# lelecaruso/NavierStokes_Project_NM4PDE

Hardware: AMD Instinct MI355X
Metric: time-steps/sec (assemble_time_step + solve_time_step), 3D flow past a cylinder, P2/P1, Yosida, per-rank ILU(0) (higher is better)
Workload: dtype f64

## Files before the change

include/nsx_host.h:

```cpp
#ifndef NSX_HOST_H
#define NSX_HOST_H

#include <stdint.h>

#ifdef __cplusplus
extern "C" {
#endif

typedef struct nsxh_mesh nsxh_mesh;
typedef struct nsxh_dofs nsxh_dofs;
typedef struct nsxh_tables nsxh_tables;


nsxh_mesh *nsxh_mesh_cylinder(int dim, int m, int nr, int nxu, int nxd, int nyb, int nyt, int nz,
                              double grade_x, double grade_r);
nsxh_mesh *nsxh_mesh_cylinder_level(int dim, int level);
nsxh_mesh *nsxh_mesh_cube(int n);
nsxh_mesh *nsxh_mesh_box(int dim, int nx, int ny, int nz, const double *lo, const double *hi);
nsxh_mesh *nsxh_mesh_read_msh(const char *path);
void nsxh_mesh_free(nsxh_mesh *);

int nsxh_mesh_dim(const nsxh_mesh *);
int nsxh_mesh_n_vertices(const nsxh_mesh *);
int nsxh_mesh_n_cells(const nsxh_mesh *);
// ... 2 lines not shown
const int32_t *nsxh_mesh_cells(const nsxh_mesh *);
const int32_t *nsxh_mesh_bfaces(const nsxh_mesh *);
const int32_t *nsxh_mesh_bface_ids(const nsxh_mesh *);
const int32_t *nsxh_mesh_bface_cells(const nsxh_mesh *);
const int32_t *nsxh_mesh_subdomain(const nsxh_mesh *);

int nsxh_mesh_partition(nsxh_mesh *, int n_parts, int n_sub);
int nsxh_mesh_partition_owned(nsxh_mesh *, int n_parts, int n_sub);


nsxh_dofs *nsxh_distribute_dofs(const nsxh_mesh *);
enum { NSXH_ORDER_FIRST_TOUCH = 0, NSXH_ORDER_COLOUR = 1, NSXH_ORDER_COLOUR_ALL = 2 };
nsxh_dofs *nsxh_distribute_dofs_ordered(const nsxh_mesh *, int ordering);
int nsxh_n_colours(const nsxh_dofs *);
int nsxh_n_colours_p(const nsxh_dofs *);
void nsxh_dofs_free(nsxh_dofs *);

int nsxh_dofs_per_cell(const nsxh_dofs *);
int nsxh_n_nodes_p2(const nsxh_dofs *);
int nsxh_n_nodes_p1(const nsxh_dofs *);
int nsxh_n_u(const nsxh_dofs *);
int nsxh_n_p(const nsxh_dofs *);
const int32_t *nsxh_cell_dofs(const nsxh_dofs *);
const double *nsxh_cell_coords(const nsxh_dofs *);
const double *nsxh_support_points(const nsxh_dofs *);
const int32_t *nsxh_node_owner(const nsxh_dofs *);
const int32_t *nsxh_pnode_owner(const nsxh_dofs *);
const int32_t *nsxh_owned_u_ptr(const nsxh_dofs *);
const int32_t *nsxh_owned_p_ptr(const nsxh_dofs *);
int nsxh_n_subdomains(const nsxh_dofs *);

int nsxh_boundary_dofs(nsxh_dofs *, int boundary_id, const int32_t **dofs);

int nsxh_reference_sparsity(nsxh_dofs *, int block, const int32_t **rowptr, const int32_t **colind);

typedef struct nsxh_rank_view nsxh_rank_view;
nsxh_rank_view *nsxh_rank_view_create(const nsxh_dofs *, int rank, int world);
void nsxh_rank_view_free(nsxh_rank_view *);
int nsxh_rank_view_n_cells(const nsxh_rank_view *);
int nsxh_rank_view_n_cells_layer1(const nsxh_rank_view *);
const int32_t *nsxh_rank_view_cell_ids(const nsxh_rank_view *);
const int32_t *nsxh_rank_view_cell_dofs(const nsxh_rank_view *);
const double *nsxh_rank_view_cell_coords(const nsxh_rank_view *);
const int32_t *nsxh_rank_view_gpu_u_ptr(const nsxh_rank_view *);
const int32_t *nsxh_rank_view_gpu_p_ptr(const nsxh_rank_view *);
int nsxh_rank_view_n_virtual_ranks(const nsxh_rank_view *);
const int32_t *nsxh_rank_view_rank_u_ptr(const nsxh_rank_view *);
const int32_t *nsxh_rank_view_rank_p_ptr(const nsxh_rank_view *);
int nsxh_rank_view_n_neighbors(const nsxh_rank_view *);
const int32_t *nsxh_rank_view_neighbors(const nsxh_rank_view *);
const int32_t *nsxh_rank_view_send_u_ptr(const nsxh_rank_view *);
const int32_t *nsxh_rank_view_send_u_nodes(const nsxh_rank_view *);
const int32_t *nsxh_rank_view_send_p_ptr(const nsxh_rank_view *);
const int32_t *nsxh_rank_view_send_p_nodes(const nsxh_rank_view *);


nsxh_tables *nsxh_tables_create(int dim, int rule, int order);
void nsxh_tables_free(nsxh_tables *);
int nsxh_tables_n_q(const nsxh_tables *);
int nsxh_tables_n_p2(const nsxh_tables *);
int nsxh_tables_n_p1(const nsxh_tables *);
const double *nsxh_tables_points(const nsxh_tables *);
const double *nsxh_tables_weights(const nsxh_tables *);
const double *nsxh_tables_N2(const nsxh_tables *);
const double *nsxh_tables_dN2(const nsxh_tables *);
const double *nsxh_tables_N1(const nsxh_tables *);
const double *nsxh_tables_dN1(const nsxh_tables *);
int nsxh_tables_n_qf(const nsxh_tables *);


int nsxh_write_vtu(const nsxh_dofs *, const double *solution, const char *directory, const char *basename, unsigned counter);

int nsxh_pressure_difference(const nsxh_dofs *, const double *solution, const double *point_a, const double *point_b, double *diff);


int nsxh_ilu_stream_stats(int n_rows, const int32_t *rowptr, const int32_t *colind, int n_blocks, const int32_t *block_ptr,
                          int blocks_per_wave, int ncomp, int gap, int entries_per_tick, int64_t out[6]);
int nsxh_ilu_stream_apply(int n_rows, const int32_t *rowptr, const int32_t *colind, int n_blocks, const int32_t *block_ptr,
                          int blocks_per_wave, int ncomp, int gap, int entries_per_tick, const double *lu, const double *b, double *x);

int nsxh_ilu_stream_apply_f32(int n_rows, const int32_t *rowptr, const int32_t *colind, int n_blocks, const int32_t *block_ptr,
                              int blocks_per_wave, int ncomp, int gap, int entries_per_tick, const double *lu, const double *b, double *x);

int nsxh_internal_layout(int dim, int n_cells, int dofs_per_cell, const int32_t *cell_dofs, const double *cell_coords, int n_u, int n_p,
                         int n_in_ranks, const int32_t *in_u_ptr, const int32_t *in_p_ptr, int n_virtual, int order, int schur_max_rows,
                         int32_t *node_perm, int32_t *pnode_perm, int32_t *n_ranks, int32_t *u_ptr, int32_t *p_ptr, int32_t *n_schur,
                         int32_t *schur_ptr, int32_t *colours);

#ifdef __cplusplus
}
#endif
#endif
```

navierstokes_project_nm4pde_amd/csrc/nsx_blas.hip:

```cpp
#include "nsx_grid.hpp"
#include "nsx_ilu_lanes.hpp"

namespace nsx {

constexpr int RED_BLOCKS = 512;
constexpr int RED_STRIDE = 1024;

struct SRef {
  double c;
  int num, den;
  int num_nb, den_nb;
};

__device__ __forceinline__ double wave_sum_all(double v) {
#pragma unroll
  for (int o = 32; o > 0; o >>= 1) v += __shfl_xor(v, o, 64);
  return v;
}

__device__ __forceinline__ double slot_value(const double *__restrict__ scal, const double *__restrict__ partial, int slot, int nb,
                                             double *sh) {
  if (nb == 0) return scal[slot];
  if (threadIdx.x < 64) {
    const double *p = partial + (size_t)slot * RED_STRIDE;
// ... 315 lines not shown
  const unsigned long long seq = ++h->pub_seq;
  unsigned long long *flag_dev = (unsigned long long *)(h->pub_dev + N_SLOTS);
  hipLaunchKernelGGL(k_publish, dim3(count), dim3(256), 0, h->stream, slot0, count, args, h->red_partial.p, h->scal.p, h->pub_dev, flag_dev, seq,
                     h->pub_counter.p);
  return seq;
}
void collect_published(nsx_handle *h, unsigned long long seq, int slot0, int count, double *out) {
  wait_published(h, seq);
  for (int i = 0; i < count; ++i) out[i] = h->pub_host[slot0 + i];
}
void read_scalars(nsx_handle *h, int slot0, int count, double *out) { collect_published(h, publish_scalars(h, slot0, count), slot0, count, out); }
void write_scalar(nsx_handle *h, int slot, double v) {
  HIP_CHECK(hipStreamSynchronize(h->stream));
  h->scal_host[slot] = v;
  h->slot_nb[slot] = 0;
  HIP_CHECK(hipMemcpyAsync(h->scal.p + slot, h->scal_host + slot, sizeof(double), hipMemcpyHostToDevice, h->stream));
  HIP_CHECK(hipStreamSynchronize(h->stream));
}

int cg_dirty_words(nsx_handle *h);

}

extern "C" int nsx_persistent_state(nsx_handle *h, int state[4]) {
  if (!h || !state) return NSX_ERR_ARG;
  try {
    HIP_CHECK(hipSetDevice(h->prm.device));
    state[0] = h->mgs.box.p != nullptr && !h->mgs.disabled && h->mgs.max_wg > 0;
    state[1] = h->cg_box.p != nullptr && !h->cg_disabled && h->cg_max_wg > 0;
    state[2] = h->n_persistent_fallbacks;
    state[3] = nsx::mgs_dirty_words(h) + nsx::cg_dirty_words(h);
  } catch (const nsx::Error &e) {
    h->err = e.msg;
    return e.code;
  }
  return NSX_OK;
}

extern "C" int nsx_path_info(nsx_handle *h, int info[32]) {
  if (!h || !info) return NSX_ERR_ARG;
  for (int k = 0; k < 32; ++k) info[k] = 0;
  if (!h->have_mesh) return NSX_OK;
  try {
    HIP_CHECK(hipSetDevice(h->prm.device));
    const nsx::SpmvBlocked &b = h->blkA;
    info[0] = nsx::blocked_usable(h) ? 1 : 0;
    info[1] = b.n_chunks;
    info[2] = b.n_chunks_if;
    info[3] = h->mgs.last_e;
    info[4] = h->mgs.last_nwg;
    info[5] = h->mgs.last_dist;
    info[6] = h->mgs.max_e_seen;
    info[7] = h->cu_reserved;
    info[8] = h->cg_last_path;
    info[9] = h->schedS.n_blocks;
    info[10] = (int)h->haloU.nbr.size();
    info[11] = h->haloU.nbr.empty() ? 0 : h->haloU.send_ptr[h->haloU.nbr.size()];
    info[12] = h->N2_loc - h->N2;
    info[13] = h->schedS.dense ? 1 : 0;
    info[14] = h->mgs.disabled ? 1 : 0;
    info[15] = h->n_persistent_fallbacks;
    if (!h->mgs.disabled) {
      nsx::mgs_setup(h);
      const int es[3] = {8, 10, 12};
      auto fit = [&](int n, const int *caps, int n_inst) {
        const nsx::MgsPick p = nsx::mgs_pick(n, caps, n_inst, es);
        return p.fits() ? p.e : 0;
      };
      info[16] = fit(h->n_u, h->mgs.max_wg_dist, 1);
      info[17] = fit(h->n_u, h->mgs.dist_cap_reserved, 3);
      info[18] = fit(h->n_u + h->n_p, h->mgs.max_wg_dist, 1);
      info[19] = fit(h->n_u + h->n_p, h->mgs.dist_cap_reserved, 3);
      info[21] = fit(h->n_u, h->mgs.max_wg_e, 3);
    }
    info[20] = nsx::cdiv(std::max(1, h->schedS.n_blocks), 1024);
    info[22] = h->N2;
    info[23] = h->NP;
    info[24] = h->mgs.last_fused;
    info[25] = h->mgs.fused_launches;
    info[26] = h->inner_F_fp32_used;
    info[27] = h->ilu_F_fp32_used;
    info[28] = h->cg_last_rpg;
    info[29] = h->cg_last_lres;
  } catch (const nsx::Error &e) {
    h->err = e.msg;
    return e.code;
  }
  return NSX_OK;
}
```

navierstokes_project_nm4pde_amd/csrc/nsx_internal.hpp:

```cpp
#pragma once
#include <hip/hip_runtime.h>

#include <cstdint>
#include <cstdio>
#include <cstring>
#include <map>
#include <string>
#include <functional>
#include <vector>

#include "../../include/nsx.h"
#include "../host/graph.hpp"

#ifndef NSX_NT
#define NSX_NT 1
#endif
template <int BIT, class T>
__device__ __forceinline__ T ld_stream(const T *p) {
  if constexpr ((NSX_NT & BIT) != 0) return __builtin_nontemporal_load(p);
  else return *p;
}

namespace nsx {

// ... 157 lines not shown
  int max_wg_e[3] = {0, 0, 0};
  int max_wg_dist[3] = {0, 0, 0};
  int dist_cap_reserved[3] = {0, 0, 0};
  int links = 0;
  bool disabled = false;
  double guard_override = -1.0;
  DevBuf<double> ls_partial, ls_vals, ls_gram;
  int ls_mode = -1;
  DevBuf<double> ext_vals;
  DevBuf<unsigned long long> ext_words;
  unsigned int ext_expected = 0;
  int ext_parity = 0;
  bool redo_ahead = false;
  int dist_state = -1;
  std::map<int, int> dist_fit;
  bool leave_req = false;
  int local_timeouts = 0;
  int ilu_cap[3] = {-1, -1, -1}, ilu_cap_rows = -1;
  int last_e = 0, last_nwg = 0, last_dist = 0, max_e_seen = 0;
  int last_fused = 0, fused_launches = 0;
};

struct Comm;

enum { N_SLOTS = 128 };

}

struct nsx_handle {
  nsx_params prm{};
  std::string err;
  hipStream_t stream = nullptr;
  int dim = 0, n_q = 0, np2 = 0, np1 = 0, dpc = 0;
  int n_cells = 0, N2 = 0, NP = 0, n_u = 0, n_p = 0;
  int N2_loc = 0, NP_loc = 0;
  int n_cells1 = 0;
  int g_u = 0, g_p = 0, off_p = 0, len_blk = 0, len_u = 0, len_p = 0;
  bool dist = false;
  int rank = 0, world = 1, goff_u = 0, goff_p = 0, n_u_glob = 0, n_p_glob = 0;
  std::vector<int32_t> ghost_u, ghost_p;
  nsx::HaloPlan haloU, haloP;
  nsx::RowSplit splitA, splitVel, splitB, splitG, splitS;
  hipStream_t comm_stream = nullptr;
  hipEvent_t ev_ready = nullptr;
  bool have_tables = false, have_mesh = false, assembled = false, prec_ready = false;
  std::vector<double> N2_h, dN2_h, N1_h, w_h;
  nsx::DevBuf<double> tab_N2, tab_dN2, tab_N1, tab_w, tab_N2T, tab_dN2T;
  nsx::DevBuf<int32_t> cell_n2, cell_n1;
  nsx::DevBuf<double> geo;
  std::vector<int32_t> cell_n2_h, cell_n1_h;
  std::vector<int32_t> cell_n2_in, cell_n1_in;
  std::vector<double> cell_coords_in;
  std::vector<int32_t> in_rank_u_h, in_rank_p_h, in_sblk_h;
  int layout_req_ranks = 0, layout_req_order = 0, layout_req_schur = 0;
  bool layout_on = false;
  int layout_colours = 0, layout_colours_p = 0;
  std::vector<int32_t> perm2_h, perm1_h, iperm2_h, iperm1_h;
  nsx::DevBuf<int32_t> perm2_d, perm1_d;
  nsx::DevBuf<double> io_stage;
  nsx::Csr caller_graph[2];
  std::vector<int32_t> caller_pos[2];
  nsx::DevCsr gA, gG, gB, gS, gPM;
  nsx::SpmvBlocked blkA;
  nsx::DevBuf<double> vS0, vMass, vStiff, vConv, vF, vG, vB, vPM, vSchur, luF, luS;
  int inner_precision = NSX_INNER_FP64;
  nsx::DevBuf<float> vF32;
  int inner_F_fp32_used = 0, ilu_F_fp32_used = 0;
  nsx::DevBuf<int32_t> bt_of_g;
  nsx::GatherMap gmA, gmG, gmB, gmPM;
  nsx::DevBuf<double> cellbuf;
  nsx::DevBuf<double> sol, sol_owned, prev_sol, rhs;
  std::vector<int32_t> rank_u_h, rank_p_h, sblk_h;
  nsx::DevBuf<int32_t> rank_u;
  nsx::IluSchedule schedF, schedS;
  nsx::DevBuf<double> dbar;
  nsx::DevBuf<int32_t> bc_dofs;
  nsx::DevBuf<double> bc_vals;
  nsx::DevBuf<double> dirmask;
  std::vector<int32_t> bc_cache;
  nsx::DevBuf<double> diag_D, diag_D_inv, neg_diag_D_inv, lump_M, schur_w;
  nsx::DevBuf<double> schur_w_prev;
  bool schur_valid = false, schur_pending = false;
  int schur_type = -1;
  std::vector<nsx::DevBuf<double> *> pool;
  nsx::DevBuf<double> red_partial;
  nsx::DevBuf<double> scal;
  int slot_nb[nsx::N_SLOTS] = {0};
  double *scal_host = nullptr;
  double *pub_host = nullptr, *pub_dev = nullptr;
  unsigned long long pub_seq = 0;
  nsx::DevBuf<unsigned int> pub_counter;
  nsx::MgsState mgs;
  bool sched_dirty = true;
  int gx_drop_wg = -1;
  int n_persistent_fallbacks = 0;
  int gmres_depth = 0;
  bool cu_reserve_failed = false;
  int cgd_agreed = -1;
  nsx::DevBuf<double> ext_self;
  hipStream_t stream_plain = nullptr;
  std::vector<hipStream_t> retired_streams;
  int cu_reserved = 0;
  int comm_probe_local = -1;
  long long n_allreduce = 0, n_halo = 0;
  int self_p2p = 0;
  int n_ext_collectives = 0;
  nsx::DevBuf<unsigned long long> cg_box;
  nsx::CgPlan cgplan;
  nsx::DevBuf<double> cg_vec;
  int cg_parity = 0, cg_max_wg = 0, cg_max_wg_res[2] = {0, 0};
  int cg_max_wg_lres[2] = {0, 0};
  bool cg_resident = false;
  bool cg_lds_resident = false;
  bool cg_variant_said = false;
  bool cg_disabled = false;
  nsx::DevBuf<double> cgd_raw;
  int cg_last_path = 0;
  int cg_last_rpg = 0, cg_last_lres = 0;
  nsx::DevBuf<double> cgd_vec, cgd_parts;
  int ff_n = 0, ff_nq = 0;
  nsx::DevBuf<int32_t> ff_cells, ff_lf;
  nsx::DevBuf<double> ff_N2, ff_dN2, ff_N1, ff_w, ff_out;
  nsx::DevBuf<uint8_t> diag_counted;
  int diag_n_counted = 0;
  nsx::DevBuf<double> diag_planes;
  nsx::DevBuf<double> diag_fold;
  nsx::DevBuf<double> diag_max;
  bool diag_valid = false;
  bool prof_on = false;
  std::map<std::string, nsx::ProfEntry> prof;
  std::vector<std::string> prof_names;
  nsx::Comm *comm = nullptr;
  bool defer_red = false;
  std::vector<int> pending_red;
};

namespace nsx {

struct LaunchScope {
  nsx_handle *h;
  ProfEntry *e = nullptr;
  hipEvent_t a = nullptr, b = nullptr;
  LaunchScope(nsx_handle *h_, const char *name, double bytes) : h(h_) {
    if (!h->prof_on) return;
    e = &h->prof[name];
    e->bytes += bytes;
    (void)hipEventCreate(&a);
    (void)hipEventCreate(&b);
    (void)hipEventRecord(a, h->stream);
  }
  ~LaunchScope() {
    if (!e) return;
    (void)hipEventRecord(b, h->stream);
    e->launches++;
    e->pending.emplace_back(a, b);
  }
};

inline int cdiv(int64_t a, int64_t b) { return (int)((a + b - 1) / b); }

void setup_ilu_schedule(nsx_handle *h, const Csr &g, const std::vector<int32_t> &block_ptr, IluSchedule &s, int blocks_per_wave, bool allow_dense = false,
                        int ncomp = 1);
void build_schur_graph(nsx_handle *h);
void vec_from_caller(nsx_handle *h, double *dev, const double *host, bool with_ghosts);
void vec_to_caller(nsx_handle *h, const double *dev, double *host);
void part_from_caller(nsx_handle *h, int which, double *dev, const double *host);
void part_to_caller(nsx_handle *h, int which, const double *dev, double *host);
void pressure_from_caller(nsx_handle *h, double *dev, const double *host);
void pressure_to_caller(nsx_handle *h, const double *dev, double *host);
inline int32_t node_to_internal(const nsx_handle *h, int32_t local_node) { return h->layout_on ? h->perm2_h[local_node] : local_node; }
inline int32_t pnode_to_internal(const nsx_handle *h, int32_t local_node) { return h->layout_on ? h->perm1_h[local_node] : local_node; }
void ensure_schedules(nsx_handle *h);

void run_assemble(nsx_handle *h, bool first, int flags);
void run_dirichlet(nsx_handle *h, int n, const int32_t *dofs, const double *vals);

void diag_mesh_setup(nsx_handle *h);

bool blocked_usable(const nsx_handle *h);
void spmv_F(nsx_handle *h, const double *vals, const double *x, double *y, const float *vals32 = nullptr, const double *rb = nullptr);
void spmv_F_inner(nsx_handle *h, const double *x, double *y);
void spmv_F_inner_resid(nsx_handle *h, const double *x, const double *b, double *y);
void convert_F_f32(nsx_handle *h);
void spmv_saddle(nsx_handle *h, const double *x, double *y);
void spmv_G(nsx_handle *h, const double *xp, double *yu, bool accumulate);
void spmv_B(nsx_handle *h, const double *xu, double *yp, const double *r = nullptr, int sub = 0);
void spmv_S(nsx_handle *h, const double *x, double *y);
void schur_numeric(nsx_handle *h, const double *w);
void ilu_factor(nsx_handle *h, const DevCsr &g, IluSchedule &s, const double *vals, double *lu, const char *name, bool f32 = false);
void ilu_check(nsx_handle *h);
bool ilu_solve(nsx_handle *h, const DevCsr &g, const IluSchedule &s, const double *lu, const double *b, double *x, int ncomp,
               const char *name, int dot_slot = -1, bool f32 = false, int *used_f32 = nullptr);
void extract_diag(nsx_handle *h, const DevCsr &g, const double *vals, double *d);
void abs_rowsum(nsx_handle *h, const DevCsr &g, const double *vals, double *d);

struct Span {
  int n, split, gap;
  Span(int n_) : n(n_), split(n_), gap(0) {}
  Span(int n_, int split_, int gap_) : n(n_), split(split_), gap(gap_) {}
};
inline Span blk_span(const nsx_handle *h) { return Span(h->n_u + h->n_p, h->n_u, h->g_u); }

template <int CTRL>
__device__ __forceinline__ double dpp_f64(double v) {
  int lo = __double2loint(v), hi = __double2hiint(v);
  lo = __builtin_amdgcn_update_dpp(0, lo, CTRL, 0xf, 0xf, true);
  hi = __builtin_amdgcn_update_dpp(0, hi, CTRL, 0xf, 0xf, true);
  return __hiloint2double(hi, lo);
}
template <int CTRL, int ROW_MASK>
__device__ __forceinline__ double dpp_f64_rows(double v) {
  int lo = __double2loint(v), hi = __double2hiint(v);
  lo = __builtin_amdgcn_update_dpp(0, lo, CTRL, ROW_MASK, 0xf, false);
  hi = __builtin_amdgcn_update_dpp(0, hi, CTRL, ROW_MASK, 0xf, false);
  return __hiloint2double(hi, lo);
}

void v_copy(nsx_handle *h, int n, double *d, const double *s);
void v_zero(nsx_handle *h, int n, double *d);
void v_add(nsx_handle *h, Span n, double *d, double a, const double *v);
void v_add_dev(nsx_handle *h, Span n, double *d, double a, int slot, const double *v);
void v_sadd(nsx_handle *h, Span n, double *d, double s, double a, const double *v);
void v_scale(nsx_handle *h, Span n, double *d, double a);
void v_scale_dev_inv(nsx_handle *h, Span n, double *d, int slot);
void v_scale_vec(nsx_handle *h, int n, double *d, const double *f);
void v_dot(nsx_handle *h, Span n, const double *a, const double *b, int slot);
void v_add_and_dot(nsx_handle *h, Span n, double *d, double a, int aslot, const double *v, const double *w, int slot);
bool v_mgs(nsx_handle *h, Span n, double *w, int dim, double *const *vs, int slot0, bool normalize, double *out,
           const std::function<void()> *after_launch = nullptr, bool consider = false, double *gram = nullptr, const double *ilu_rhs = nullptr);
void v_axpy_multi(nsx_handle *h, Span n, double *x, int k, double *const *vs, const double *coef_host);
void v_axpy_multi_into(nsx_handle *h, Span n, double *x, const double *x0, const double *y, int k, double *const *vs, const double *coef_host);
void finalize_slots(nsx_handle *h, int slot0, int count);
double *red_out(nsx_handle *h, int slot, int nb);
void after_reduction(nsx_handle *h, int slot, int nb);
int red_blocks(nsx_handle *h, int n);
__device__ __forceinline__ double block_sum_256(double v, double *sh) {
#pragma unroll
  for (int o = 32; o > 0; o >>= 1) v += __shfl_down(v, o, 64);
  const int w = threadIdx.x >> 6, l = threadIdx.x & 63;
  if (l == 0) sh[w] = v;
  __syncthreads();
  double t = 0.0;
  if (threadIdx.x == 0) {
    for (int k = 0; k < (int)(blockDim.x >> 6); ++k) t += sh[k];
  }
  return t;
}
void defer_reductions(nsx_handle *h, bool on);
double read_scalar(nsx_handle *h, int slot);
void read_scalars(nsx_handle *h, int slot0, int count, double *out);
unsigned long long publish_scalars(nsx_handle *h, int slot0, int count);
void collect_published(nsx_handle *h, unsigned long long seq, int slot0, int count, double *out);
void wait_published(nsx_handle *h, unsigned long long seq);
void mgs_setup(nsx_handle *h);
int mgs_dirty_words(nsx_handle *h);
struct MgsPick {
  int e = 0, nwg = 1, per_thread = 1 << 30;
  bool fits() const { return e != 0 && per_thread <= e; }
};
MgsPick mgs_pick(int n, const int *caps, int n_inst, const int *es);
void build_cg_plan(nsx_handle *h);
void cg_pack_values(nsx_handle *h);
bool cg_schur_persistent(nsx_handle *h, double *x, const double *b, double rtol, int maxiter, int *steps, double *last, int *status);
bool cg_schur_fused(nsx_handle *h, double *x, const double *b, double rtol, int maxiter, int *steps, double *last, int *status);
void write_scalar(nsx_handle *h, int slot, double v);

void prec_initialize(nsx_handle *h, int type);
void prec_confirm(nsx_handle *h);
void prec_vmult(nsx_handle *h, int type, double inner_rtol, int inner_maxiter, double *dst, const double *src,
                nsx_solve_stats *st, bool fused);
void solve_time_step(nsx_handle *h, int type, double tol, double inner_rtol, int maxiter, int inner_maxiter,
                     nsx_solve_stats *st);

void comm_allreduce_scalars(nsx_handle *h, int slot0, int count);
void comm_allreduce_partials(nsx_handle *h, double *partials, int count);
bool comm_agree_all(nsx_handle *h, bool mine);
// ... 17 lines not shown
```

navierstokes_project_nm4pde_amd/csrc/nsx_setup.hip:

```cpp
#include <algorithm>
#include <cmath>
#include <numeric>

#include "nsx_internal.hpp"
#include "../host/ilu_stream.hpp"
#include "../host/layout.hpp"

using namespace nsx;

static thread_local std::string g_create_error;

namespace nsx {

static void upload_csr(nsx_handle *h, DevCsr &d, bool square) {
  d.rowptr.upload(d.host.rowptr, h->stream);
  d.colind.upload(d.host.colind, h->stream);
  if (square) {
    std::vector<int32_t> diag(d.host.n_rows);
    for (int32_t i = 0; i < d.host.n_rows; ++i) {
      diag[i] = find_in_row(d.host, i, i);
      if (diag[i] < 0) NSX_THROW(NSX_ERR_ARG, "square graph has no diagonal entry in row %d", i);
    }
    d.diag.upload(diag, h->stream);
  }
}

static void build_gather(nsx_handle *h, const Csr &g, int n_cells, int per_r, const int32_t *cell_r, int per_c,
                         const int32_t *cell_c, int plane_stride, bool plane_rc_swapped, GatherMap &gm) {
  const int64_t nnz = g.nnz();
  std::vector<int32_t> ptr(nnz + 1, 0);
  std::vector<int32_t> epos((size_t)n_cells * per_r * per_c);
  for (int c = 0; c < n_cells; ++c)
    for (int a = 0; a < per_r; ++a)
      for (int b = 0; b < per_c; ++b) {
        const int32_t row = cell_r[(size_t)c * per_r + a];
        if (row >= g.n_rows) {
          epos[((size_t)c * per_r + a) * per_c + b] = -1;
          continue;
        }
        const int32_t e = find_in_row(g, row, cell_c[(size_t)c * per_c + b]);
        if (e < 0) NSX_THROW(NSX_ERR_ARG, "internal: cell pair not in graph");
        epos[((size_t)c * per_r + a) * per_c + b] = e;
        ptr[e + 1]++;
      }
  for (int64_t e = 0; e < nnz; ++e) ptr[e + 1] += ptr[e];
  std::vector<int32_t> src(ptr[nnz]);
  std::vector<int32_t> fill(ptr.begin(), ptr.end() - 1);
  for (int c = 0; c < n_cells; ++c)
    for (int a = 0; a < per_r; ++a)
      for (int b = 0; b < per_c; ++b) {
        const int32_t e = epos[((size_t)c * per_r + a) * per_c + b];
        if (e < 0) continue;
        const int64_t plane = plane_rc_swapped ? ((int64_t)b * per_r + a) : ((int64_t)a * per_c + b);
        const int64_t off = plane * plane_stride * n_cells + c;
        if (off > INT32_MAX) NSX_THROW(NSX_ERR_UNSUPPORTED, "mesh too large for int32 gather offsets");
        src[fill[e]++] = (int32_t)off;
      }
  gm.n_out = nnz;
  gm.n_src = (int64_t)src.size();
  gm.ptr.upload(ptr, h->stream);
  gm.src.upload(src, h->stream);
}

void setup_ilu_schedule(nsx_handle *h, const Csr &g, const std::vector<int32_t> &bptr, IluSchedule &s, int blocks_per_wave, bool allow_dense, int ncomp) {
  const int nb = (int)bptr.size() - 1;
  s.n_blocks = nb;
  s.block_ptr_h = bptr;
  s.max_rows = 0;
  std::vector<int32_t> lev(g.n_rows, 0);
  std::vector<int32_t> f_ptr{0}, f_rows, b_ptr{0}, b_rows, off_f(nb + 1, 0), off_b(nb + 1, 0);
  f_rows.reserve(g.n_rows);
  b_rows.reserve(g.n_rows);
  s.max_levels = 0;
  std::vector<std::vector<int32_t>> buckets;
  for (int b = 0; b < nb; ++b) {
    const int r0 = bptr[b], r1 = bptr[b + 1];
    s.max_rows = std::max(s.max_rows, r1 - r0);
    for (int pass = 0; pass < 2; ++pass) {
      int nl = 0;
      if (pass == 0) {
        for (int i = r0; i < r1; ++i) {
          int l = 0;
          for (int k = g.rowptr[i]; k < g.rowptr[i + 1]; ++k) {
            const int j = g.colind[k];
            if (j >= i) break;
            if (j >= r0) l = std::max(l, lev[j] + 1);
          }
          lev[i] = l;
          nl = std::max(nl, l + 1);
// ... 214 lines not shown
    b.grid_if = 0;
    b.frac_if = g.nnz() ? (double)nnz_second / (double)g.nnz() : 0.0;
    if (!second.empty()) make_desc(second, b.desc_if, b.grid_if, nullptr);
  }
  b.crow.upload(bounds, h->stream);
  b.cptr.upload(cptr, h->stream);
  b.ucols.upload(ucols, h->stream);
  b.lidx.upload(lidx, h->stream);
  if (getenv("NSX_DEBUG"))
    fprintf(stderr, "[nsx] blocked spmv: rows %d chunks %d (max %d rows; %d of them stage a ghost column: %.1f %% of the non-zeros) unique cols/chunk avg %.0f max %d (nnz/unique %.1f)\n",
            g.n_rows, b.n_chunks, b.max_rows, b.n_chunks_if, 100.0 * b.frac_if, b.ucols_total / std::max(1, b.n_chunks), b.max_ucols, (double)g.nnz() / b.ucols_total);
}

static std::vector<int32_t> spmv_chunks(nsx_handle *h) {
  const int n = h->gA.host.n_rows;
  const int target = getenv("NSX_SPMV_R") ? std::max(16, std::min(448, atoi(getenv("NSX_SPMV_R")))) : 130;
  std::vector<int32_t> bounds{0};
  const std::vector<int32_t> &rk = h->rank_u_h;
  const bool by_rank = !(getenv("NSX_SPMV_BY_RANK") && atoi(getenv("NSX_SPMV_BY_RANK")) == 0) && rk.size() > 2 &&
                       (double)n / (double)(rk.size() - 1) <= target;
  const bool split_ranks = !by_rank && !(getenv("NSX_SPMV_BY_RANK") && atoi(getenv("NSX_SPMV_BY_RANK")) == 0) && rk.size() > 2 &&
                           (double)n / (double)(rk.size() - 1) <= 4.0 * target;
  if (by_rank) {
    int start = 0;
    for (size_t r = 1; r < rk.size(); ++r) {
      if (rk[r] - start > target && rk[r - 1] > start) {
        bounds.push_back(rk[r - 1]);
        start = rk[r - 1];
      }
    }
    bounds.push_back(n);
  } else if (split_ranks) {
    for (size_t r = 0; r + 1 < rk.size(); ++r) {
      const int rows = rk[r + 1] - rk[r];
      if (rows <= 0) continue;
      const int parts = (rows + target - 1) / target;
      for (int q = 1; q <= parts; ++q) bounds.push_back(rk[r] + (int)((int64_t)rows * q / parts));
    }
    if (bounds.back() != n) bounds.push_back(n);
  } else {
    for (int r = 128; r < n; r += 128) bounds.push_back(r);
    bounds.push_back(n);
  }
  std::vector<int32_t> out{0};
  for (size_t c = 1; c < bounds.size(); ++c) {
    while (bounds[c] - out.back() > 448) out.push_back(out.back() + 224);
    if (bounds[c] > out.back()) out.push_back(bounds[c]);
  }
  return out;
}

void build_schur_graph(nsx_handle *h) {
  const Csr &B = h->gB.host;
  std::vector<int32_t> tp((size_t)h->N2_loc + 1, 0), tr(B.nnz());
  for (int64_t k = 0; k < B.nnz(); ++k) tp[B.colind[k] + 1]++;
  for (int i = 0; i < h->N2_loc; ++i) tp[i + 1] += tp[i];
  {
    std::vector<int32_t> fill(tp.begin(), tp.end() - 1);
    for (int j = 0; j < B.n_rows; ++j)
      for (int k = B.rowptr[j]; k < B.rowptr[j + 1]; ++k) tr[fill[B.colind[k]]++] = j;
  }
  Csr S;
  S.n_rows = h->NP;
  S.n_cols = h->NP_loc;
  S.rowptr.assign((size_t)h->NP + 1, 0);
  std::vector<int32_t> mark(h->NP_loc, -1), cols;
  for (int i = 0; i < h->NP; ++i) {
    cols.clear();
    for (int kb = B.rowptr[i]; kb < B.rowptr[i + 1]; ++kb) {
      const int k = B.colind[kb];
      for (int q = tp[k]; q < tp[k + 1]; ++q) {
        const int j = tr[q];
        if (mark[j] != i) {
          mark[j] = i;
          cols.push_back(j);
        }
      }
    }
    std::sort(cols.begin(), cols.end());
    S.colind.insert(S.colind.end(), cols.begin(), cols.end());
    S.rowptr[i + 1] = (int32_t)S.colind.size();
  }
  h->gS.host = std::move(S);
  upload_csr(h, h->gS, true);
  h->vSchur.alloc(h->gS.nnz());
  h->luS.alloc(h->gS.nnz());
}

static void default_ranks(nsx_handle *h) {
  h->in_rank_u_h = {0, h->N2};
  h->in_rank_p_h = {0, h->NP};
  h->in_sblk_h.clear();
}

static void refresh_rank_products(nsx_handle *h) {
  h->rank_u.upload(h->rank_u_h, h->stream);
  h->dbar.alloc(h->rank_u_h.size() - 1);
  h->sched_dirty = true;
  h->prec_ready = false;
  h->schur_valid = false;
  h->mgs.dist_fit.clear();
}

void ensure_schedules(nsx_handle *h) {
  if (!h->sched_dirty) return;
  build_blocked(h, h->gA.host, spmv_chunks(h), h->blkA, h->N2);
  auto blocks_per_wave = [](int n_rows, size_t n_blocks) { return std::max(1, std::min(64, (int)(680.0 * (double)n_blocks / std::max(1, n_rows) + 0.5))); };
  const std::vector<int32_t> &sb = h->sblk_h.empty() ? h->rank_p_h : h->sblk_h;
  const int bpwF = getenv("NSX_BPW_F") ? atoi(getenv("NSX_BPW_F")) : blocks_per_wave(h->N2, h->rank_u_h.size() - 1);
  const int bpwS = getenv("NSX_BPW_S") ? atoi(getenv("NSX_BPW_S")) : blocks_per_wave(h->NP, sb.size() - 1);
  setup_ilu_schedule(h, h->gA.host, h->rank_u_h, h->schedF, bpwF, false, h->dim);
  const bool denseS = !(getenv("NSX_DENSE_S") && atoi(getenv("NSX_DENSE_S")) == 0);
  setup_ilu_schedule(h, h->gS.host, sb, h->schedS, bpwS, denseS, 1);
  build_cg_plan(h);
  h->cgd_agreed = -1;
  h->sched_dirty = false;
}


__global__ void k_perm_vec(int n, int ncomp, const int32_t *__restrict__ perm, double *caller, double *internal, int to_internal) {
  const int i = blockIdx.x * blockDim.x + threadIdx.x;
  if (i >= n) return;
  const int node = i / ncomp, c = i - node * ncomp;
  const int64_t j = (int64_t)perm[node] * ncomp + c;
  if (to_internal) internal[j] = caller[i];
  else caller[i] = internal[j];
}

static void perm_launch(nsx_handle *h, int which, double *caller_dev, double *internal_dev, bool to_internal) {
  const int ncomp = which == 0 ? h->dim : 1, n = which == 0 ? h->n_u : h->n_p;
  if (n) hipLaunchKernelGGL(k_perm_vec, dim3(cdiv(n, 256)), dim3(256), 0, h->stream, n, ncomp, (which == 0 ? h->perm2_d : h->perm1_d).p, caller_dev, internal_dev, to_internal ? 1 : 0);
}

void part_from_caller(nsx_handle *h, int which, double *dev, const double *host) {
  const int n = which == 0 ? h->n_u : h->n_p;
  if (!h->layout_on) {
    HIP_CHECK(hipMemcpyAsync(dev, host, (size_t)n * sizeof(double), hipMemcpyHostToDevice, h->stream));
  } else {
    h->io_stage.alloc((size_t)h->n_u + h->n_p);
    HIP_CHECK(hipMemcpyAsync(h->io_stage.p, host, (size_t)n * sizeof(double), hipMemcpyHostToDevice, h->stream));
    perm_launch(h, which, h->io_stage.p, dev, true);
  }
  HIP_CHECK(hipStreamSynchronize(h->stream));
}

void part_to_caller(nsx_handle *h, int which, const double *dev, double *host) {
  const int n = which == 0 ? h->n_u : h->n_p;
  if (!h->layout_on) {
    HIP_CHECK(hipMemcpyAsync(host, dev, (size_t)n * sizeof(double), hipMemcpyDeviceToHost, h->stream));
  } else {
    h->io_stage.alloc((size_t)h->n_u + h->n_p);
    perm_launch(h, which, h->io_stage.p, const_cast<double *>(dev), false);
    HIP_CHECK(hipMemcpyAsync(host, h->io_stage.p, (size_t)n * sizeof(double), hipMemcpyDeviceToHost, h->stream));
  }
  HIP_CHECK(hipStreamSynchronize(h->stream));
}

void pressure_from_caller(nsx_handle *h, double *dev, const double *host) {
  if (!h->dist) return part_from_caller(h, 1, dev, host);
  std::vector<double> loc(h->len_p, 0.0);
  for (int i = 0; i < h->NP; ++i) loc[pnode_to_internal(h, i)] = host[(size_t)h->goff_p + i];
  HIP_CHECK(hipMemcpyAsync(dev, loc.data(), loc.size() * sizeof(double), hipMemcpyHostToDevice, h->stream));
  HIP_CHECK(hipStreamSynchronize(h->stream));
}
void pressure_to_caller(nsx_handle *h, const double *dev, double *host) {
  if (!h->dist) return part_to_caller(h, 1, dev, host);
  std::vector<double> loc(h->n_p);
  HIP_CHECK(hipMemcpyAsync(loc.data(), dev, loc.size() * sizeof(double), hipMemcpyDeviceToHost, h->stream));
  HIP_CHECK(hipStreamSynchronize(h->stream));
  for (int i = 0; i < h->NP; ++i) host[(size_t)h->goff_p + i] = loc[pnode_to_internal(h, i)];
}

void vec_from_caller(nsx_handle *h, double *dev, const double *host, bool with_ghosts) {
  const int dim = h->dim;
  if (!h->dist) {
    if (!h->layout_on) {
      HIP_CHECK(hipMemcpyAsync(dev, host, ((size_t)h->n_u + h->n_p) * sizeof(double), hipMemcpyHostToDevice, h->stream));
    } else {
      h->io_stage.alloc((size_t)h->n_u + h->n_p);
      HIP_CHECK(hipMemcpyAsync(h->io_stage.p, host, ((size_t)h->n_u + h->n_p) * sizeof(double), hipMemcpyHostToDevice, h->stream));
      perm_launch(h, 0, h->io_stage.p, dev, true);
      perm_launch(h, 1, h->io_stage.p + h->n_u, dev + h->off_p, true);
    }
    HIP_CHECK(hipStreamSynchronize(h->stream));
    return;
  }
  std::vector<double> loc(h->len_blk, 0.0);
  for (int i = 0; i < h->N2; ++i)
    for (int c = 0; c < dim; ++c) loc[(size_t)dim * node_to_internal(h, i) + c] = host[(size_t)dim * (h->goff_u + i) + c];
  for (int i = 0; i < h->NP; ++i) loc[h->off_p + pnode_to_internal(h, i)] = host[(size_t)h->n_u_glob + h->goff_p + i];
  if (with_ghosts) {
    for (size_t g = 0; g < h->ghost_u.size(); ++g)
      for (int c = 0; c < dim; ++c) loc[h->n_u + g * dim + c] = host[(size_t)dim * h->ghost_u[g] + c];
    for (size_t g = 0; g < h->ghost_p.size(); ++g) loc[h->off_p + h->n_p + g] = host[(size_t)h->n_u_glob + h->ghost_p[g]];
  }
  HIP_CHECK(hipMemcpyAsync(dev, loc.data(), loc.size() * sizeof(double), hipMemcpyHostToDevice, h->stream));
  HIP_CHECK(hipStreamSynchronize(h->stream));
// ... 773 lines not shown
```

navierstokes_project_nm4pde_amd/csrc/nsx_solve.hip:

```cpp
#include <chrono>
#include <cmath>
#include <functional>
#include <memory>

#include "nsx_internal.hpp"

namespace nsx {

void cg_update(nsx_handle *h, int n, double *x, const double *d, double *g, const double *hv, int gh_slot, int dh_slot, int res_slot);
void cg_direction(nsx_handle *h, int n, double *d, const double *hv, int num_slot, int den_slot);
void v_reciprocal(nsx_handle *h, int n, double *d, const double *s, double num);

struct Tmp {
  nsx_handle *h;
  DevBuf<double> *b;
  Tmp(nsx_handle *h_, size_t n) : h(h_), b(nullptr) {
    for (size_t i = 0; i < h->pool.size(); ++i)
      if (h->pool[i]->n >= n) {
        b = h->pool[i];
        h->pool.erase(h->pool.begin() + i);
        break;
      }
    if (!b) {
      b = new DevBuf<double>();
// ... 221 lines not shown
}

using OpDot = std::function<bool(double *dst, const double *src, int slot)>;
static SolveResult cg(nsx_handle *h, const Op &A, double *x, const double *b, const Op &P, Span n, int len, double tol, int maxiter,
                      const OpDot *Pdot = nullptr) {
  auto apply_P_dot = [&](double *dst, const double *src, int slot) {
    if (Pdot && (*Pdot)(dst, src, slot)) return;
    if (!Pdot) P(dst, src);
    v_dot(h, n, src, dst, slot);
  };
  SolveResult res{1, 0, 0.0};
  Tmp g(h, len), d(h, len), hv(h, len);
  int it = 0;
  A(g.p(), x);
  v_add(h, n, g.p(), -1., b);
  v_dot(h, n, g.p(), g.p(), S_RES);
  double r = std::sqrt(read_scalar(h, S_RES));
  res.last = r;
  int conv = sc_check(0, r, tol, maxiter);
  if (conv == 0) {
    int gh = S_GH, gh_new = S_GH2;
    apply_P_dot(hv.p(), g.p(), gh);
    v_copy(h, n.n, d.p(), hv.p());
    v_scale(h, n, d.p(), -1.);
    while (conv == 0) {
      it++;
      A(hv.p(), d.p());
      v_dot(h, n, d.p(), hv.p(), S_DH);
      const bool batch = h->comm != nullptr;
      DeferScope defer(h, batch);
      cg_update(h, n.n, x, d.p(), g.p(), hv.p(), gh, S_DH, S_RES);
      unsigned long long seq = 0;
      if (!batch) seq = publish_scalars(h, S_RES, 1);
      apply_P_dot(hv.p(), g.p(), gh_new);
      if (batch) {
        defer.release();
        seq = publish_scalars(h, S_RES, 1);
      }
      double res2;
      collect_published(h, seq, S_RES, 1, &res2);
      r = std::sqrt(std::fabs(res2));
      res.last = r;
      conv = sc_check(it, r, tol, maxiter);
      if (conv != 0) break;
      cg_direction(h, n.n, d.p(), hv.p(), gh_new, gh);
      std::swap(gh, gh_new);
    }
  }
  res.status = conv == 1 ? 0 : 1;
  res.steps = it;
  return res;
}

static double norm2(nsx_handle *h, Span n, const double *v) {
  v_dot(h, n, v, v, S_T);
  return std::sqrt(read_scalar(h, S_T));
}

static Op schur_product(nsx_handle *h) {
  return [h](double *d, const double *s) { spmv_S(h, s, d); };
}
static Op schur_ilu(nsx_handle *h) {
  return [h](double *d, const double *s) { ilu_solve(h, h->gS, h->schedS, h->luS.p, s, d, 1, "ilu_solve_S"); };
}

static SolveResult schur_cg(nsx_handle *h, double rtol, int maxit, double *x, const double *b) {
  int steps = 0, status = 0;
  double last = 0.0;
  h->cg_last_rpg = h->cg_last_lres = 0;
  if (cg_schur_persistent(h, x, b, rtol, maxit, &steps, &last, &status)) return SolveResult{status, steps, last};
  if (cg_schur_fused(h, x, b, rtol, maxit, &steps, &last, &status)) return SolveResult{status, steps, last};
  h->cg_last_path = 1;
  const Op Sm = schur_product(h), PS = schur_ilu(h);
  OpDot PSdot = [h](double *d, const double *s, int slot) { return ilu_solve(h, h->gS, h->schedS, h->luS.p, s, d, 1, "ilu_solve_S", slot); };
  return cg(h, Sm, x, b, PS, h->n_p, h->len_p, rtol * norm2(h, h->n_p, b), maxit, &PSdot);
}

__global__ void k_same_and_keep(int n, const double *__restrict__ w, double *__restrict__ prev, int *changed) {
  const int i = blockIdx.x * blockDim.x + threadIdx.x;
  if (i >= n) return;
  const unsigned long long a = (unsigned long long)__double_as_longlong(w[i]), b = (unsigned long long)__double_as_longlong(prev[i]);
  if (a != b) {
    prev[i] = w[i];
    __hip_atomic_store(changed, 1, __ATOMIC_RELAXED, __HIP_MEMORY_SCOPE_SYSTEM);
  }
}
static bool schur_inputs_unchanged(nsx_handle *h, int type) {
  const bool cache = !(getenv("NSX_SCHUR_CACHE") && atoi(getenv("NSX_SCHUR_CACHE")) == 0);
  const int n = h->len_u;
  volatile int *flag = (volatile int *)(h->pub_host + N_SLOTS + 4);
  const bool had = h->schur_valid && h->schur_type == type && (int)h->schur_w_prev.n == n;
  if (!had) {
    h->schur_w_prev.alloc(n);
    comm_halo_u(h, h->schur_w.p);
    v_copy(h, n, h->schur_w_prev.p, h->schur_w.p);
    return false;
  }
  comm_halo_u(h, h->schur_w.p);
  *flag = 0;
  hipLaunchKernelGGL(k_same_and_keep, dim3(cdiv(n, 256)), dim3(256), 0, h->stream, n, h->schur_w.p, h->schur_w_prev.p, (int *)(h->pub_dev + N_SLOTS + 4));
  HIP_CHECK(hipStreamSynchronize(h->stream));
  return cache && !h->comm && *flag == 0;
}

void prec_initialize(nsx_handle *h, int type) {
  ensure_schedules(h);
  if (!h->assembled) NSX_THROW(NSX_ERR_ARG, "assemble before initialising a preconditioner");
  HIP_CHECK(hipSetDevice(h->prm.device));
  const int n_u = h->n_u;
  const double *V = nullptr;
  if (type == NSX_PREC_YOSIDA) {
    extract_diag(h, h->gA, h->vMass.p, h->diag_D.p);
  } else if (type == NSX_PREC_SIMPLE || type == NSX_PREC_ASIMPLE || type == NSX_PREC_AYOSIDA) {
    extract_diag(h, h->gA, h->vF.p, h->diag_D.p);
  } else {
    NSX_THROW(NSX_ERR_ARG, "Invalid preconditioner type");
  }
  v_reciprocal(h, n_u, h->diag_D_inv.p, h->diag_D.p, 1.0);
  v_reciprocal(h, n_u, h->neg_diag_D_inv.p, h->diag_D.p, -1.0);
  V = h->neg_diag_D_inv.p;
  if (type == NSX_PREC_AYOSIDA) {
    abs_rowsum(h, h->gA, h->vMass.p, h->lump_M.p);
    v_reciprocal(h, n_u, h->lump_M.p, h->lump_M.p, -1.0);
    V = h->lump_M.p;
  }
  v_copy(h, n_u, h->schur_w.p, V);
  v_scale_vec(h, n_u, h->schur_w.p, h->dirmask.p);
  v_scale(h, n_u, h->schur_w.p, -1.0);
  const bool f32 = h->inner_precision == NSX_INNER_FP32;
  if (f32) convert_F_f32(h);
  ilu_factor(h, h->gA, h->schedF, h->vF.p, h->luF.p, "ilu_factor_F", f32);
  if (!schur_inputs_unchanged(h, type)) {
    h->schur_valid = false;
    h->schur_pending = true;
    schur_numeric(h, h->schur_w.p);
    cg_pack_values(h);
    ilu_factor(h, h->gS, h->schedS, h->vSchur.p, h->luS.p, "ilu_factor_S");
    h->schur_type = type;
  }
  h->prec_ready = true;
}

void prec_confirm(nsx_handle *h) {
  try {
    ilu_check(h);
  } catch (...) {
    h->schur_valid = false;
    h->schur_pending = false;
    h->prec_ready = false;
    throw;
  }
  if (h->schur_pending) {
    h->schur_pending = false;
    h->schur_valid = true;
  }
}

static void count(nsx_solve_stats *st, bool F, const SolveResult &r) {
  if (!st) return;
  if (F) {
    st->inner_F_iterations += r.steps;
    st->n_F_solves++;
  } else {
    st->inner_S_iterations += r.steps;
    st->n_S_solves++;
  }
  if (r.status) st->status = 2;
}

static bool step_fused() { return !(getenv("NSX_STEP_FUSED") && atoi(getenv("NSX_STEP_FUSED")) == 0); }

void prec_vmult(nsx_handle *h, int type, double tol, int maxit, double *dst, const double *src, nsx_solve_stats *st, bool fused) {
  if (!h->prec_ready) NSX_THROW(NSX_ERR_ARG, "preconditioner not initialised");
  const int n_u = h->n_u, n_p = h->n_p, dim = h->dim, len_u = h->len_u, len_p = h->len_p;
  const double *src_u = src, *src_p = src + h->off_p;
  double *dst_u = dst, *dst_p = dst + h->off_p;
  Op Fm = [h](double *d, const double *s) { spmv_F_inner(h, s, d); };
  const bool f32 = h->inner_precision == NSX_INNER_FP32;
  const Op Sm = schur_product(h), PS = schur_ilu(h);
  Op PF = [h, dim, f32](double *d, const double *s) {
    int used = 0;
    ilu_solve(h, h->gA, h->schedF, h->luF.p, s, d, dim, "ilu_solve_F", -1, f32, &used);
    if (used) h->ilu_F_fp32_used = 1;
  };
  auto cg_S = [&](double *x, const double *b) { return schur_cg(h, tol, maxit, x, b); };
  const ResidOp Fr = [h](double *d, const double *x, const double *b) { spmv_F_inner_resid(h, x, b, d); };
  auto solve_F = [&](double *x, const double *b, bool x_is_zero, Seams *sm) {
    if (!sm) return count(st, true, gmres(h, Fm, x, b, PF, n_u, len_u, tol * norm2(h, n_u, b), maxit, false, x_is_zero, true, true));
    sm->rtol = tol;
    sm->A_resid = &Fr;
    v_dot(h, n_u, b, b, S_T);
    count(st, true, gmres(h, Fm, x, b, PF, n_u, len_u, 0.0, maxit, false, x_is_zero, true, true, sm));
  };
  auto solve_F_from_src = [&](double *x) {
    if (!fused) return solve_F(x, src_u, false, nullptr);
    Seams sm;
    sm.x0 = src_u;
    solve_F(x, src_u, false, &sm);
    if (!sm.x_written) v_copy(h, n_u, x, src_u);
  };
  auto B_and_sub = [&](const double *x, double *out, const double *r, int sign) {
    if (fused) return spmv_B(h, x, out, r, sign);
    spmv_B(h, x, out);
    if (sign > 0) v_add(h, n_p, out, -1.0, r);
    else v_sadd(h, n_p, out, -1.0, 1.0, r);
  };
  std::unique_ptr<Tmp> own_u, own_p;
  double *yu = dst_u, *yp = dst_p;
  if (!fused && (type == NSX_PREC_YOSIDA || type == NSX_PREC_SIMPLE)) {
    own_u = std::make_unique<Tmp>(h, len_u);
    own_p = std::make_unique<Tmp>(h, len_p);
    yu = own_u->p();
    yp = own_p->p();
  }
// ... 245 lines not shown
```

navierstokes_project_nm4pde_amd/csrc/nsx_sparse.hip:

```cpp
#include <atomic>

#include "nsx_internal.hpp"
#include "nsx_ilu_lanes.hpp"

namespace nsx {

template <int LW>
__device__ __forceinline__ double lane_group_sum(double v) {
  if (LW >= 2) v += dpp_f64<0xB1>(v);
  if (LW >= 4) v += dpp_f64<0x4E>(v);
  if (LW >= 8) v += dpp_f64<0x141>(v);
  if (LW >= 16) v += dpp_f64<0x140>(v);
  if (LW >= 32) v += __shfl_xor(v, 16, 64);
  if (LW >= 64) v += __shfl_xor(v, 32, 64);
  return v;
}

template <int W>
__device__ __forceinline__ double group_sum(double v) {
  return lane_group_sum<W>(v);
}

template <int DIM, int W, bool WITH_G, bool RESID>
__device__ __forceinline__ void spmv_vel_rows(int n_rows, const int32_t *__restrict__ rp, const int32_t *__restrict__ ci,
                                              const double *__restrict__ av, const double *__restrict__ x,
                                              const int32_t *__restrict__ grp, const int32_t *__restrict__ gci,
                                              const double *__restrict__ gv, const double *__restrict__ xp,
                                              double *__restrict__ y, const int32_t *__restrict__ rows, const double *__restrict__ b) {
  const int bid = (blockIdx.x & 7) * (gridDim.x >> 3) + (blockIdx.x >> 3);
  const int slot = (bid * 256 + threadIdx.x) / W, lane = threadIdx.x % W;
  if (slot >= n_rows) return;
  const int row = rows ? rows[slot] : slot;
  double acc[DIM];
#pragma unroll
  for (int c = 0; c < DIM; ++c) acc[c] = 0.0;
  const int e = rp[row + 1];
  for (int p = rp[row] + lane; p < e; p += W) {
    const double a = av[p];
    const double *xj = x + (size_t)ci[p] * DIM;
#pragma unroll
    for (int c = 0; c < DIM; ++c) acc[c] += a * xj[c];
  }
  if (WITH_G) {
    const int ge = grp[row + 1];
    for (int p = grp[row] + lane; p < ge; p += W) {
      const double xk = xp[gci[p]];
#pragma unroll
      for (int c = 0; c < DIM; ++c) acc[c] += gv[(size_t)p * DIM + c] * xk;
    }
  }
#pragma unroll
  for (int c = 0; c < DIM; ++c) acc[c] = group_sum<W>(acc[c]);
  if (lane == 0) {
#pragma unroll
    for (int c = 0; c < DIM; ++c) y[(size_t)row * DIM + c] = RESID ? b[(size_t)row * DIM + c] - acc[c] : acc[c];
  }
}
template <int DIM, int W, bool WITH_G>
__global__ __launch_bounds__(256) void k_spmv_vel(int n_rows, const int32_t *__restrict__ rp, const int32_t *__restrict__ ci,
                                                  const double *__restrict__ av, const double *__restrict__ x,
                                                  const int32_t *__restrict__ grp, const int32_t *__restrict__ gci,
                                                  const double *__restrict__ gv, const double *__restrict__ xp,
                                                  double *__restrict__ y, const int32_t *__restrict__ rows) {
  spmv_vel_rows<DIM, W, WITH_G, false>(n_rows, rp, ci, av, x, grp, gci, gv, xp, y, rows, nullptr);
}
template <int DIM, int W>
__global__ __launch_bounds__(256) void k_spmv_vel_resid(int n_rows, const int32_t *__restrict__ rp, const int32_t *__restrict__ ci,
                                                        const double *__restrict__ av, const double *__restrict__ x, double *__restrict__ y,
                                                        const int32_t *__restrict__ rows, const double *__restrict__ b) {
  spmv_vel_rows<DIM, W, false, true>(n_rows, rp, ci, av, x, nullptr, nullptr, nullptr, nullptr, y, rows, b);
}

template <int DIM, int W>
__global__ __launch_bounds__(256) void k_spmv_G(int n_rows, const int32_t *__restrict__ rp, const int32_t *__restrict__ ci,
                                                const double *__restrict__ gv, const double *__restrict__ xp,
                                                double *__restrict__ y, int accumulate, const int32_t *__restrict__ rows) {
  const int slot = (blockIdx.x * 256 + threadIdx.x) / W, lane = threadIdx.x % W;
  if (slot >= n_rows) return;
  const int row = rows ? rows[slot] : slot;
  double acc[DIM];
#pragma unroll
  for (int c = 0; c < DIM; ++c) acc[c] = 0.0;
  const int e = rp[row + 1];
  for (int p = rp[row] + lane; p < e; p += W) {
    const double xk = xp[ci[p]];
#pragma unroll
// ... 389 lines not shown

void spmv_saddle(nsx_handle *h, const double *x, double *y) {
  double *xx = const_cast<double *>(x);
  if (h->dist) {
    comm_halo_begin(h, h->haloU, xx, h->dim);
    comm_halo_begin(h, h->haloP, xx + h->off_p, 1);
  }
  const bool blk_dist = h->dist && blocked_usable(h);
  {
    LaunchScope ls(h, "spmv_saddle_u", bytes_vel(h, true));
    if (blk_dist) launch_blocked(h, h->vF.p, x, y, 0);
    else if (h->dist) launch_vel(h, true, h->vF.p, x, x + h->off_p, y, h->splitVel.interior.p, h->splitVel.n_interior);
    else if (launch_blocked(h, h->vF.p, x, y)) launch_G(h, x + h->off_p, y, true, nullptr, h->N2);
    else launch_vel(h, true, h->vF.p, x, x + h->off_p, y, nullptr, h->N2);
  }
  {
    LaunchScope ls(h, "spmv_B", bytes_B(h));
    if (h->dist) launch_B(h, x, y + h->off_p, h->splitB.interior.p, h->splitB.n_interior);
    else launch_B(h, x, y + h->off_p, nullptr, h->NP);
  }
  if (h->dist) {
    {
      LaunchScope ls(h, "halo_up_wait", bytes_halo(h->haloU, h->dim) + bytes_halo(h->haloP, 1));
      comm_halo_finish(h, h->haloU, xx, h->dim);
      comm_halo_finish(h, h->haloP, xx + h->off_p, 1);
    }
    LaunchScope ls(h, "spmv_saddle_if", 0);
    if (blk_dist) {
      launch_blocked(h, h->vF.p, x, y, 1);
      launch_G(h, x + h->off_p, y, true, nullptr, h->N2);
    } else {
      launch_vel(h, true, h->vF.p, x, x + h->off_p, y, h->splitVel.interface.p, h->splitVel.n_interface);
    }
    launch_B(h, x, y + h->off_p, h->splitB.interface.p, h->splitB.n_interface);
  }
}

void spmv_S(nsx_handle *h, const double *x, double *y) {
  LaunchScope ls(h, "spmv_S", 12.0 * h->gS.nnz() + 20.0 * h->NP);
  if (h->dist) {
    double *xx = const_cast<double *>(x);
    comm_halo_begin(h, h->haloP, xx, 1);
    launch_S(h, x, y, h->splitS.interior.p, h->splitS.n_interior);
    comm_halo_finish(h, h->haloP, xx, 1);
    launch_S(h, x, y, h->splitS.interface.p, h->splitS.n_interface);
    return;
  }
  launch_S(h, x, y, nullptr, h->NP);
}

static void split_rows(nsx_handle *h, RowSplit &sp, int n_rows, const Csr &a, int own_a, const Csr *b, int own_b) {
  std::vector<int32_t> in, out;
  for (int i = 0; i < n_rows; ++i) {
    bool ghost = false;
    for (int k = a.rowptr[i]; k < a.rowptr[i + 1] && !ghost; ++k) ghost = a.colind[k] >= own_a;
    if (b)
      for (int k = b->rowptr[i]; k < b->rowptr[i + 1] && !ghost; ++k) ghost = b->colind[k] >= own_b;
    (ghost ? out : in).push_back(i);
  }
  sp.n_interior = (int)in.size();
  sp.n_interface = (int)out.size();
  sp.interior.upload(in, h->stream);
  sp.interface.upload(out, h->stream);
}
void build_row_splits(nsx_handle *h) {
  if (!h->dist) return;
  split_rows(h, h->splitA, h->N2, h->gA.host, h->N2, nullptr, 0);
  split_rows(h, h->splitVel, h->N2, h->gA.host, h->N2, &h->gG.host, h->NP);
  split_rows(h, h->splitG, h->N2, h->gG.host, h->NP, nullptr, 0);
  split_rows(h, h->splitB, h->NP, h->gB.host, h->N2, nullptr, 0);
  split_rows(h, h->splitS, h->NP, h->gS.host, h->NP, nullptr, 0);
  if (getenv("NSX_DEBUG"))
    fprintf(stderr, "[nsx] rank %d: interface rows F %d / %d, block(1,0) %d / %d, S %d / %d\n", h->rank, h->splitA.n_interface, h->N2, h->splitB.n_interface,
            h->NP, h->splitS.n_interface, h->NP);
}

void convert_F_f32(nsx_handle *h) {
  const int64_t n = h->gA.nnz();
  h->vF32.alloc((size_t)n);
  LaunchScope ls(h, "F_to_f32", 12.0 * (double)n);
  if (n > 0) hipLaunchKernelGGL(k_to_f32, dim3(cdiv(n, 256)), dim3(256), 0, h->stream, n, h->vF.p, h->vF32.p, (int *)(h->pub_dev + N_SLOTS + 3));
}

__global__ void k_extract_diag(int n_nodes, int dim, const int32_t *__restrict__ diag, const double *__restrict__ v, double *__restrict__ d) {
  const int i = blockIdx.x * blockDim.x + threadIdx.x;
  if (i >= n_nodes * dim) return;
  d[i] = v[diag[i / dim]];
}
__global__ void k_abs_rowsum(int n_nodes, int dim, const int32_t *__restrict__ rp, const double *__restrict__ v, double *__restrict__ d) {
  const int i = blockIdx.x * blockDim.x + threadIdx.x;
  if (i >= n_nodes) return;
  double s = 0.0;
  for (int p = rp[i]; p < rp[i + 1]; ++p) s += fabs(v[p]);
  for (int c = 0; c < dim; ++c) d[(size_t)i * dim + c] = s;
}
void extract_diag(nsx_handle *h, const DevCsr &g, const double *vals, double *d) {
  LaunchScope ls(h, "extract_diag", 0);
  hipLaunchKernelGGL(k_extract_diag, dim3(cdiv(h->n_u, 256)), dim3(256), 0, h->stream, g.n_rows(), h->dim, g.diag.p, vals, d);
}
void abs_rowsum(nsx_handle *h, const DevCsr &g, const double *vals, double *d) {
  LaunchScope ls(h, "abs_rowsum", 0);
  hipLaunchKernelGGL(k_abs_rowsum, dim3(cdiv(g.n_rows(), 256)), dim3(256), 0, h->stream, g.n_rows(), h->dim, g.rowptr.p, vals, d);
}

template <int DIM>
__global__ __launch_bounds__(64) void k_schur(int n_rows, const int32_t *__restrict__ srp, const int32_t *__restrict__ sci,
                                              const int32_t *__restrict__ brp, const int32_t *__restrict__ bci,
                                              const double *__restrict__ bv, const double *__restrict__ w, int max_row,
                                              double *__restrict__ sv) {
  extern __shared__ double smem[];
  double *rv = smem;
  int32_t *rc = (int32_t *)(smem + (size_t)max_row * DIM);
  const int i = blockIdx.x;
  if (i >= n_rows) return;
  const int b0 = brp[i], nb = brp[i + 1] - b0;
  for (int t = threadIdx.x; t < nb; t += 64) {
    const int k = bci[b0 + t];
    rc[t] = k;
#pragma unroll
    for (int c = 0; c < DIM; ++c) rv[t * DIM + c] = bv[(size_t)(b0 + t) * DIM + c] * w[(size_t)k * DIM + c];
  }
  __syncthreads();
  for (int e = srp[i] + threadIdx.x; e < srp[i + 1]; e += 64) {
    const int j = sci[e];
    double acc = 0.0;
    int q = 0;
    for (int p = brp[j]; p < brp[j + 1]; ++p) {
      const int k = bci[p];
      while (q < nb && rc[q] < k) ++q;
      if (q < nb && rc[q] == k) {
#pragma unroll
        for (int c = 0; c < DIM; ++c) acc += rv[q * DIM + c] * bv[(size_t)p * DIM + c];
      }
    }
    sv[e] = acc;
  }
}

void schur_numeric(nsx_handle *h, const double *w) {
  comm_halo_u(h, w);
  int max_row = 0;
  const Csr &B = h->gB.host;
  for (int i = 0; i < B.n_rows; ++i) max_row = std::max(max_row, B.rowptr[i + 1] - B.rowptr[i]);
  const size_t shm = (size_t)max_row * (h->dim * 8 + 4) + 8;
  if (shm > 160 * 1024) NSX_THROW(NSX_ERR_UNSUPPORTED, "row of block(1,0) too long for the Schur kernel (%d)", max_row);
  LaunchScope ls(h, "schur_numeric", 0);
  if (h->dim == 2)
    hipLaunchKernelGGL((k_schur<2>), dim3(h->NP), dim3(64), shm, h->stream, h->NP, h->gS.rowptr.p, h->gS.colind.p, h->gB.rowptr.p,
                       h->gB.colind.p, h->vB.p, w, max_row, h->vSchur.p);
  else
    hipLaunchKernelGGL((k_schur<3>), dim3(h->NP), dim3(64), shm, h->stream, h->NP, h->gS.rowptr.p, h->gS.colind.p, h->gB.rowptr.p,
                       h->gB.colind.p, h->vB.p, w, max_row, h->vSchur.p);
}

constexpr int ILU_WAVES = 4;
constexpr int ILU_MAXROW = 1024;

__device__ __forceinline__ void pk_store(double *__restrict__ pk_val, float *__restrict__ pk_val32, int sl, double v, int *err) {
  if (pk_val32) {
    const float f = (float)v;
    pk_val32[sl] = f;
    if (!(fabsf(f) <= 3.402823466e+38f)) __hip_atomic_store(err, 5, __ATOMIC_RELAXED, __HIP_MEMORY_SCOPE_SYSTEM);
  } else {
    pk_val[sl] = v;
  }
}

__global__ __launch_bounds__(ILU_WAVES * 64) void k_ilu_factor(const int32_t *__restrict__ bptr, const int32_t *__restrict__ lvl_off,
                                                              const int32_t *__restrict__ lvl_ptr, const int32_t *__restrict__ lvl_rows,
                                                              const int32_t *__restrict__ rp, const int32_t *__restrict__ ci,
                                                              const int32_t *__restrict__ diag, const double *__restrict__ a,
                                                              double *__restrict__ lu, const int32_t *__restrict__ slot_of,
                                                              double *__restrict__ pk_val, double *__restrict__ pk_dinv,
                                                              int *__restrict__ err, const int32_t *__restrict__ dinv_slot,
                                                              float *__restrict__ pk_val32) {
  __shared__ double wv[ILU_WAVES][ILU_MAXROW];
  const int blk = blockIdx.x, wave = threadIdx.x / 64, lane = threadIdx.x % 64;
  const int r0 = bptr[blk], r1 = bptr[blk + 1];
  volatile double *w = wv[wave];
  for (int lv = lvl_off[blk]; lv < lvl_off[blk + 1]; ++lv) {
    const int l0 = lvl_ptr[lv], cnt = lvl_ptr[lv + 1] - l0;
    for (int r = wave; r < cnt; r += ILU_WAVES) {
      const int i = lvl_rows[l0 + r];
      const int p0 = rp[i], n = rp[i + 1] - p0, dpos = diag[i] - p0;
      if (n > ILU_MAXROW) {
        if (lane == 0) __hip_atomic_store(err, 1, __ATOMIC_RELAXED, __HIP_MEMORY_SCOPE_SYSTEM);
        continue;
      }
      for (int t = lane; t < n; t += 64) {
        const int j = ci[p0 + t];
        w[t] = (j >= r0 && j < r1) ? a[p0 + t] : 0.0;
      }
      __builtin_amdgcn_wave_barrier();
      for (int t = 0; t < dpos; ++t) {
        const int j = ci[p0 + t];
        if (j < r0) continue;
        const int dj = diag[j];
        const double mult = w[t];
        __builtin_amdgcn_wave_barrier();
        if (lane == 0) w[t] = mult * lu[dj];
        const int ue = rp[j + 1];
        for (int q = dj + 1 + lane; q < ue; q += 64) {
          const int c = ci[q];
          if (c >= r1) break;
          int lo = t + 1, hi = n - 1;
          while (lo <= hi) {
            const int mid = (lo + hi) >> 1, cm = ci[p0 + mid];
            if (cm < c) lo = mid + 1; else if (cm > c) hi = mid - 1; else { w[mid] -= mult * lu[q]; break; }
          }
        }
        __builtin_amdgcn_wave_barrier();
      }
      const double d = w[dpos];
      const double dinv = 1.0 / d;
      if (lane == 0 && !(fabs(d) > 0.0)) __hip_atomic_store(err, 2, __ATOMIC_RELAXED, __HIP_MEMORY_SCOPE_SYSTEM);
      for (int t = lane; t < n; t += 64) {
        const int j = ci[p0 + t];
        double v = w[t];
        if (t == dpos) v = dinv;
        else if (t > dpos) v = (j < r1) ? v * dinv : 0.0;
        lu[p0 + t] = v;
        if (slot_of) {
          const int sl = slot_of[p0 + t];
          if (sl >= 0) pk_store(pk_val, pk_val32, sl, -v, err);
          if (t == dpos) pk_dinv[dinv_slot[i]] = dinv;
        }
      }
      __builtin_amdgcn_wave_barrier();
    }
    __syncthreads();
  }
}

__global__ __launch_bounds__(128) void k_ilu_invert_lds(const int32_t *__restrict__ bptr, const int64_t *__restrict__ off,
                                                        const int32_t *__restrict__ rp, const int32_t *__restrict__ ci,
                                                        const int32_t *__restrict__ diag, const double *__restrict__ lu, double *__restrict__ P) {
  extern __shared__ double Ps[];
  __shared__ int s_rp[113], s_dg[112];
  const int blk = blockIdx.x, r0 = bptr[blk], n = bptr[blk + 1] - r0;
  const int j = threadIdx.x;
  for (int t = threadIdx.x; t <= n; t += 128) s_rp[t] = rp[r0 + t];
  for (int t = threadIdx.x; t < n; t += 128) s_dg[t] = diag[r0 + t];
  __syncthreads();
  if (j < n) {
    for (int i = 0; i < n; ++i) {
      const int pe = s_dg[i];
      double acc = i == j ? 1.0 : 0.0;
      for (int p = s_rp[i]; p < pe; ++p) {
        const int k = ci[p] - r0;
        if (k >= 0) acc -= lu[p] * Ps[k * n + j];
      }
      Ps[i * n + j] = acc;
    }
    for (int i = n - 1; i >= 0; --i) {
      const int pd = s_dg[i], pe = s_rp[i + 1];
      double acc = lu[pd] * Ps[i * n + j];
      for (int p = pd + 1; p < pe; ++p) {
        const int k = ci[p] - r0;
        if (k < n) acc -= lu[p] * Ps[k * n + j];
      }
      Ps[i * n + j] = acc;
    }
  }
  __syncthreads();
  double *Pb = P + off[blk];
  for (int q = threadIdx.x; q < n * n; q += 128) Pb[q] = Ps[q];
}

__global__ __launch_bounds__(256) void k_ilu_invert(const int32_t *__restrict__ bptr, const int64_t *__restrict__ off,
                                                    const int32_t *__restrict__ rp, const int32_t *__restrict__ ci,
                                                    const int32_t *__restrict__ diag, const double *__restrict__ lu, double *P) {
  const int blk = blockIdx.x, r0 = bptr[blk], n = bptr[blk + 1] - r0;
  double *Pb = P + off[blk];
  for (int j = threadIdx.x; j < n; j += 256) {
    for (int i = 0; i < n; ++i) {
      const int row = r0 + i, pe = diag[row];
      double acc = i == j ? 1.0 : 0.0;
      for (int p = rp[row]; p < pe; ++p) {
        const int k = ci[p] - r0;
        if (k >= 0) acc -= lu[p] * Pb[(size_t)k * n + j];
      }
      Pb[(size_t)i * n + j] = acc;
    }
    for (int i = n - 1; i >= 0; --i) {
      const int row = r0 + i, pd = diag[row], pe = rp[row + 1];
      double acc = lu[pd] * Pb[(size_t)i * n + j];
      for (int p = pd + 1; p < pe; ++p) {
        const int k = ci[p] - r0;
        if (k < n) acc -= lu[p] * Pb[(size_t)k * n + j];
      }
      Pb[(size_t)i * n + j] = acc;
    }
  }
}

constexpr int DENSE_THREADS = 1024;
__global__ __launch_bounds__(DENSE_THREADS) void k_ilu_apply_dense(const int32_t *__restrict__ bptr, const int64_t *__restrict__ off,
                                                                   const double *__restrict__ P, const double *b, double *x,
                                                                   double *__restrict__ dot_partial) {
  extern __shared__ double bs[];
  __shared__ double sh[DENSE_THREADS / 64];
  const int blk = blockIdx.x, r0 = bptr[blk], n = bptr[blk + 1] - r0;
  const double *Pb = P + off[blk];
  for (int t = threadIdx.x; t < n; t += DENSE_THREADS) bs[t] = b[r0 + t];
  __syncthreads();
  const int grp = threadIdx.x >> 4, lane = threadIdx.x & 15;
  double dot = 0.0;
  for (int i = grp; i < n; i += DENSE_THREADS / 16) {
    const double *row = Pb + (size_t)i * n;
    double a0 = 0.0, a1 = 0.0;
    int j = lane;
    for (; j + 16 < n; j += 32) {
      a0 += row[j] * bs[j];
      a1 += row[j + 16] * bs[j + 16];
    }
    if (j < n) a0 += row[j] * bs[j];
    const double acc = lane_group_sum<16>(a0 + a1);
    if (lane == 0) {
      x[r0 + i] = acc;
      dot += bs[i] * acc;
    }
  }
  if (dot_partial) {
    dot = lane_group_sum<64>(dot);
    if ((threadIdx.x & 63) == 0) sh[threadIdx.x >> 6] = dot;
    __syncthreads();
    if (threadIdx.x == 0) {
      double t = 0.0;
#pragma unroll
      for (int k = 0; k < DENSE_THREADS / 64; ++k) t += sh[k];
      dot_partial[blk] = t;
    }
  }
}

constexpr int ILU_DENSE_ROWS = 512;
__global__ __launch_bounds__(ILU_WAVES * 64) void k_ilu_factor_small(const int32_t *__restrict__ bptr, const int32_t *__restrict__ lvl_off,
                                                                    const int32_t *__restrict__ lvl_ptr, const int32_t *__restrict__ lvl_rows,
                                                                    const int32_t *__restrict__ rp, const int32_t *__restrict__ ci,
                                                                    const int32_t *__restrict__ diag, const double *__restrict__ a,
                                                                    double *__restrict__ lu, const int32_t *__restrict__ slot_of,
                                                                    double *__restrict__ pk_val, double *__restrict__ pk_dinv,
                                                                    int *__restrict__ err, const int32_t *__restrict__ dinv_slot,
                                                                    float *__restrict__ pk_val32) {
// ... 244 lines not shown
  }
#pragma unroll
  for (int c = 0; c < NCOMP; ++c) acc[c] = lane_group_sum<LW>(acc[c]);
  if (lane == 0) {
#pragma unroll
    for (int c = 0; c < NCOMP; ++c) xi[c] = FWD ? xi0[c] - acc[c] : xi0[c] * dinv - acc[c];
  }
}

template <int NCOMP>
static void ilu_solve_levelled(nsx_handle *h, const DevCsr &g, const IluSchedule &s, const double *lu, const double *b, double *x) {
  constexpr int LW = 8;
  v_copy(h, g.n_rows() * NCOMP, x, b);
  const int nf = (int)s.gl_f_ptr_h.size() - 1, nbk = (int)s.gl_b_ptr_h.size() - 1;
  for (int l = 1; l < nf; ++l) {
    const int n = s.gl_f_ptr_h[l + 1] - s.gl_f_ptr_h[l];
    if (n > 0)
      hipLaunchKernelGGL((k_ilu_solve_level<NCOMP, LW, true>), dim3(cdiv((int64_t)n * LW, 256)), dim3(256), 0, h->stream, n,
                         reinterpret_cast<const int4 *>(s.gl_f_rec.p) + s.gl_f_ptr_h[l], g.colind.p, lu, x);
  }
  for (int l = 0; l < nbk; ++l) {
    const int n = s.gl_b_ptr_h[l + 1] - s.gl_b_ptr_h[l];
    if (n > 0)
      hipLaunchKernelGGL((k_ilu_solve_level<NCOMP, LW, false>), dim3(cdiv((int64_t)n * LW, 256)), dim3(256), 0, h->stream, n,
                         reinterpret_cast<const int4 *>(s.gl_b_rec.p) + s.gl_b_ptr_h[l], g.colind.p, lu, x);
  }
}

void ilu_check(nsx_handle *h) {
  volatile int *err = (volatile int *)(h->pub_host + N_SLOTS + 3);
  const int herr = *err;
  if (!herr) return;
  *err = 0;
  if (herr == 1) NSX_THROW(NSX_ERR_UNSUPPORTED, "ILU: a row has more than %d entries", ILU_MAXROW);
  if (herr == 3) NSX_THROW(NSX_ERR_HIP, "ILU: the lane-owner triangular solve found its LDS array away from address 0 and did not run (internal: a static __shared__ object in k_ilu_solve_lanes?)");
  if (herr == 4) NSX_THROW(NSX_ERR_NUMERIC, "inner precision FP32: an entry of F is not finite as a float (beyond 3.4e38, or NaN)");
  if (herr == 5) NSX_THROW(NSX_ERR_NUMERIC, "inner precision FP32: an entry of the ILU(0) factors of F is not finite as a float (beyond 3.4e38, or NaN)");
  NSX_THROW(NSX_ERR_NUMERIC, "ILU: zero pivot");
}

void ilu_factor(nsx_handle *h, const DevCsr &g, IluSchedule &s, const double *vals, double *lu, const char *name, bool f32) {
  int *err = (int *)(h->pub_dev + N_SLOTS + 3);
  float *pk32 = nullptr;
  if (f32 && ilu_lanes_stream(s, s.stream_ncomp)) {
    if (s.pk_val32.n != s.pk_val.n || !s.pk_val32.p) {
      s.pk_val32.alloc(s.pk_val.n);
      s.pk_val32.zero(h->stream);
    }
    pk32 = s.pk_val32.p;
  }
  s.stream_f32 = pk32 != nullptr;
  {
    LaunchScope ls(h, name, 20.0 * g.nnz() + 12.0 * g.n_rows());
    static const bool small_ok = !(getenv("NSX_ILU_SMALL") && atoi(getenv("NSX_ILU_SMALL")) == 0);
    const bool lds_ok = !(getenv("NSX_ILU_FACTOR_LDS") && atoi(getenv("NSX_ILU_FACTOR_LDS")) == 0);
    if (s.levelled) {
      for (size_t l = 0; l + 1 < s.gl_f_ptr_h.size(); ++l) {
        const int n = s.gl_f_ptr_h[l + 1] - s.gl_f_ptr_h[l];
        if (n > 0)
          hipLaunchKernelGGL(k_ilu_factor_level, dim3(cdiv(n, ILU_WAVES)), dim3(ILU_WAVES * 64), 0, h->stream, n, s.gl_f_rows.p + s.gl_f_ptr_h[l],
                             s.in_lo.p, s.in_hi.p, g.rowptr.p, g.colind.p, g.diag.p, vals, lu, err);
      }
    } else if (lds_ok && s.max_rows <= 4096 && s.max_block_nnz < 65535 && ilu_factor_lds_bytes(s.max_rows, s.max_block_nnz) <= 80 * 1024) {
      const size_t lds = ilu_factor_lds_bytes(s.max_rows, s.max_block_nnz);
      static std::atomic<size_t> lds_allowed{64 * 1024};
      if (lds > lds_allowed.load()) {
        HIP_CHECK(hipFuncSetAttribute((const void *)k_ilu_factor_lds, hipFuncAttributeMaxDynamicSharedMemorySize, 80 * 1024));
        lds_allowed.store(80 * 1024);
      }
      hipLaunchKernelGGL(k_ilu_factor_lds, dim3(s.n_blocks), dim3(ILU_WAVES * 64), lds, h->stream, s.fac_order.p, s.block_ptr.p, s.blk_lvl_off.p, s.fwd_lvl_ptr.p,
                         s.fwd_rows.p, g.rowptr.p, g.colind.p, g.diag.p, s.in_lo.p, s.in_cptr.p, s.in_cpos.p, vals, lu,
                         s.packed_ok ? s.pk_slot_of.p : nullptr, s.pk_val.p, s.pk_dinv.p, err, s.pk_dinv_slot.p, s.max_rows, (int)s.max_block_nnz, pk32);
    } else if (small_ok && s.max_rows <= ILU_DENSE_ROWS)
      hipLaunchKernelGGL(k_ilu_factor_small, dim3(s.n_blocks), dim3(ILU_WAVES * 64), 0, h->stream, s.block_ptr.p, s.blk_lvl_off.p,
                         s.fwd_lvl_ptr.p, s.fwd_rows.p, g.rowptr.p, g.colind.p, g.diag.p, vals, lu, s.packed_ok ? s.pk_slot_of.p : nullptr,
                         s.pk_val.p, s.pk_dinv.p, err, s.pk_dinv_slot.p, pk32);
    else
      hipLaunchKernelGGL(k_ilu_factor, dim3(s.n_blocks), dim3(ILU_WAVES * 64), 0, h->stream, s.block_ptr.p, s.blk_lvl_off.p, s.fwd_lvl_ptr.p,
                         s.fwd_rows.p, g.rowptr.p, g.colind.p, g.diag.p, vals, lu, s.packed_ok ? s.pk_slot_of.p : nullptr, s.pk_val.p,
                         s.pk_dinv.p, err, s.pk_dinv_slot.p, pk32);
  }
  if (s.dense) {
    LaunchScope ls(h, "ilu_invert", 8.0 * (double)s.dn_entries + 12.0 * g.nnz());
    const bool inv_lds = !(getenv("NSX_ILU_INVERT_LDS") && atoi(getenv("NSX_ILU_INVERT_LDS")) == 0);
    const size_t shm = (size_t)s.max_rows * s.max_rows * sizeof(double);
    if (inv_lds && s.max_rows <= 112) {
      static bool attr_set = false;
      if (!attr_set && shm > 64 * 1024) {
        HIP_CHECK(hipFuncSetAttribute((const void *)k_ilu_invert_lds, hipFuncAttributeMaxDynamicSharedMemorySize, 112 * 112 * (int)sizeof(double)));
        attr_set = true;
      }
      hipLaunchKernelGGL(k_ilu_invert_lds, dim3(s.n_blocks), dim3(128), shm, h->stream, s.block_ptr.p, s.dn_off.p, g.rowptr.p, g.colind.p, g.diag.p, lu, s.dn_P.p);
    } else {
      hipLaunchKernelGGL(k_ilu_invert, dim3(s.n_blocks), dim3(256), 0, h->stream, s.block_ptr.p, s.dn_off.p, g.rowptr.p, g.colind.p, g.diag.p, lu,
                         s.dn_P.p);
    }
  }
}

template <int NCOMP, int LW, bool USE_LDS>
__global__ __launch_bounds__(256) void k_ilu_solve(const int32_t *__restrict__ bptr, const int32_t *__restrict__ offF,
                                                   const int32_t *__restrict__ ptrF, const int32_t *__restrict__ rowsF,
                                                   const int32_t *__restrict__ offB, const int32_t *__restrict__ ptrB,
                                                   const int32_t *__restrict__ rowsB, const int32_t *__restrict__ rp,
                                                   const int32_t *__restrict__ ci, const int32_t *__restrict__ diag,
                                                   const double *__restrict__ lu, const double *__restrict__ b, double *__restrict__ x) {
  extern __shared__ double xs_[];
  const int blk = blockIdx.x;
  const int r0 = bptr[blk], r1 = bptr[blk + 1], nloc = r1 - r0;
  double *xs = USE_LDS ? xs_ : x + (size_t)r0 * NCOMP;
  for (int t = threadIdx.x; t < nloc * NCOMP; t += 256) xs[t] = b[(size_t)r0 * NCOMP + t];
  __syncthreads();
  const int grp = threadIdx.x / LW, lane = threadIdx.x % LW, ngrp = 256 / LW;
  for (int lv = offF[blk]; lv < offF[blk + 1]; ++lv) {
    const int l0 = ptrF[lv], cnt = ptrF[lv + 1] - l0;
    for (int r = grp; r < cnt; r += ngrp) {
      const int i = rowsF[l0 + r];
      double acc[NCOMP];
#pragma unroll
      for (int c = 0; c < NCOMP; ++c) acc[c] = 0.0;
      const int e = diag[i];
      for (int p = rp[i] + lane; p < e; p += LW) {
        const int j = ci[p];
        if (j >= r0) {
          const double l = lu[p];
#pragma unroll
          for (int c = 0; c < NCOMP; ++c) acc[c] += l * xs[(j - r0) * NCOMP + c];
        }
      }
#pragma unroll
      for (int c = 0; c < NCOMP; ++c) acc[c] = group_sum<LW>(acc[c]);
      if (lane == 0) {
#pragma unroll
        for (int c = 0; c < NCOMP; ++c) xs[(i - r0) * NCOMP + c] -= acc[c];
      }
    }
    __syncthreads();
  }
  for (int t = threadIdx.x; t < nloc; t += 256) {
    const double dinv = lu[diag[r0 + t]];
#pragma unroll
    for (int c = 0; c < NCOMP; ++c) xs[t * NCOMP + c] *= dinv;
  }
  __syncthreads();
  for (int lv = offB[blk]; lv < offB[blk + 1]; ++lv) {
    const int l0 = ptrB[lv], cnt = ptrB[lv + 1] - l0;
    for (int r = grp; r < cnt; r += ngrp) {
      const int i = rowsB[l0 + r];
      double acc[NCOMP];
#pragma unroll
      for (int c = 0; c < NCOMP; ++c) acc[c] = 0.0;
      const int e = rp[i + 1];
      for (int p = diag[i] + 1 + lane; p < e; p += LW) {
        const int j = ci[p];
        if (j < r1) {
          const double u = lu[p];
#pragma unroll
          for (int c = 0; c < NCOMP; ++c) acc[c] += u * xs[(j - r0) * NCOMP + c];
        }
      }
#pragma unroll
      for (int c = 0; c < NCOMP; ++c) acc[c] = group_sum<LW>(acc[c]);
      if (lane == 0) {
#pragma unroll
        for (int c = 0; c < NCOMP; ++c) xs[(i - r0) * NCOMP + c] -= acc[c];
      }
    }
    __syncthreads();
  }
  if (USE_LDS)
    for (int t = threadIdx.x; t < nloc * NCOMP; t += 256) x[(size_t)r0 * NCOMP + t] = xs[t];
}

constexpr int LANES_K = 12;

template <int NCOMP, int E, int PF, class VT>
__device__ __forceinline__ void ilu_solve_lanes_wave(const int32_t *__restrict__ row_ptr, const int32_t *__restrict__ rows,
                                                     const int32_t *__restrict__ slab_ptr, const uint32_t *__restrict__ meta,
// ... 214 lines not shown
```

navierstokes_project_nm4pde_amd/frontend.py:

```python
import ctypes as C

import numpy as np

from ._lib import HOST_SO, load

_i32p = C.POINTER(C.c_int32)
_f64p = C.POINTER(C.c_double)


def _lib():
    lib = load(HOST_SO)
    if getattr(lib, "_nsxh_ready", False):
        return lib
    vp = C.c_void_p
    sig = {
        "nsxh_mesh_cylinder": (vp, [C.c_int] * 8 + [C.c_double] * 2),
        "nsxh_mesh_cylinder_level": (vp, [C.c_int, C.c_int]),
        "nsxh_mesh_cube": (vp, [C.c_int]),
        "nsxh_mesh_box": (vp, [C.c_int] * 4 + [_f64p, _f64p]),
        "nsxh_mesh_read_msh": (vp, [C.c_char_p]),
        "nsxh_mesh_free": (None, [vp]),
        "nsxh_mesh_dim": (C.c_int, [vp]),
        "nsxh_mesh_n_vertices": (C.c_int, [vp]),
        "nsxh_mesh_n_cells": (C.c_int, [vp]),
        "nsxh_mesh_n_bfaces": (C.c_int, [vp]),
        "nsxh_mesh_vertices": (_f64p, [vp]),
        "nsxh_mesh_cells": (_i32p, [vp]),
        "nsxh_mesh_bfaces": (_i32p, [vp]),
        "nsxh_mesh_bface_ids": (_i32p, [vp]),
        "nsxh_mesh_bface_cells": (_i32p, [vp]),
        "nsxh_mesh_subdomain": (_i32p, [vp]),
        "nsxh_mesh_partition": (C.c_int, [vp, C.c_int, C.c_int]),
        "nsxh_mesh_partition_owned": (C.c_int, [vp, C.c_int, C.c_int]),
        "nsxh_distribute_dofs": (vp, [vp]),
        "nsxh_distribute_dofs_ordered": (vp, [vp, C.c_int]),
        "nsxh_n_colours": (C.c_int, [vp]),
        "nsxh_n_colours_p": (C.c_int, [vp]),
        "nsxh_write_vtu": (C.c_int, [vp, C.POINTER(C.c_double), C.c_char_p, C.c_char_p, C.c_uint]),
        "nsxh_pressure_difference": (C.c_int, [vp, C.POINTER(C.c_double), C.POINTER(C.c_double), C.POINTER(C.c_double), C.POINTER(C.c_double)]),
        "nsxh_dofs_free": (None, [vp]),
        "nsxh_dofs_per_cell": (C.c_int, [vp]),
        "nsxh_n_nodes_p2": (C.c_int, [vp]),
        "nsxh_n_nodes_p1": (C.c_int, [vp]),
        "nsxh_n_u": (C.c_int, [vp]),
        "nsxh_n_p": (C.c_int, [vp]),
        "nsxh_cell_dofs": (_i32p, [vp]),
        "nsxh_cell_coords": (_f64p, [vp]),
        "nsxh_support_points": (_f64p, [vp]),
        "nsxh_node_owner": (_i32p, [vp]),
        "nsxh_pnode_owner": (_i32p, [vp]),
        "nsxh_owned_u_ptr": (_i32p, [vp]),
        "nsxh_owned_p_ptr": (_i32p, [vp]),
        "nsxh_n_subdomains": (C.c_int, [vp]),
        "nsxh_boundary_dofs": (C.c_int, [vp, C.c_int, C.POINTER(_i32p)]),
        "nsxh_reference_sparsity": (C.c_int, [vp, C.c_int, C.POINTER(_i32p), C.POINTER(_i32p)]),
        "nsxh_tables_create": (vp, [C.c_int, C.c_int, C.c_int]),
        "nsxh_tables_free": (None, [vp]),
        "nsxh_tables_n_q": (C.c_int, [vp]),
        "nsxh_tables_n_qf": (C.c_int, [vp]),
        "nsxh_tables_n_p2": (C.c_int, [vp]),
        "nsxh_tables_n_p1": (C.c_int, [vp]),
        "nsxh_tables_points": (_f64p, [vp]),
        "nsxh_tables_weights": (_f64p, [vp]),
        "nsxh_tables_N2": (_f64p, [vp]),
        "nsxh_tables_dN2": (_f64p, [vp]),
        "nsxh_tables_N1": (_f64p, [vp]),
        "nsxh_tables_dN1": (_f64p, [vp]),
        "nsxh_ilu_stream_stats": (C.c_int, [C.c_int, _i32p, _i32p, C.c_int, _i32p, C.c_int, C.c_int, C.c_int, C.c_int, C.POINTER(C.c_int64)]),
        "nsxh_ilu_stream_apply": (C.c_int, [C.c_int, _i32p, _i32p, C.c_int, _i32p, C.c_int, C.c_int, C.c_int, C.c_int, _f64p, _f64p, _f64p]),
        "nsxh_ilu_stream_apply_f32": (C.c_int, [C.c_int, _i32p, _i32p, C.c_int, _i32p, C.c_int, C.c_int, C.c_int, C.c_int, _f64p, _f64p, _f64p]),
        "nsxh_internal_layout": (C.c_int, [C.c_int, C.c_int, C.c_int, _i32p, _f64p, C.c_int, C.c_int, C.c_int, _i32p, _i32p, C.c_int, C.c_int, C.c_int,
                                           _i32p, _i32p, _i32p, _i32p, _i32p, _i32p, _i32p, _i32p]),
    }
    for name, (res, args) in sig.items():
        fn = getattr(lib, name)
        fn.restype = res
        fn.argtypes = args
    lib._nsxh_ready = True
    return lib


def _arr(ptr, shape, dtype, copy=True):
    n = int(np.prod(shape))
    if n == 0:
        return np.zeros(shape, dtype=dtype)
    nbytes = n * np.dtype(dtype).itemsize
    buf = (C.c_char * nbytes).from_address(C.cast(ptr, C.c_void_p).value)
    a = np.frombuffer(buf, dtype=dtype, count=n).reshape(shape)
    return a.copy() if copy else a


class Mesh:

    def __init__(self, handle):
        if not handle:
            raise ValueError("mesh construction failed (bad parameters or unreadable file)")
        self._h = handle
        self._lib = _lib()
        self.refresh()

    def refresh(self):
        L, h = self._lib, self._h
        self.dim = L.nsxh_mesh_dim(h)
        nv, nc, nb = L.nsxh_mesh_n_vertices(h), L.nsxh_mesh_n_cells(h), L.nsxh_mesh_n_bfaces(h)
        self.vertices = _arr(L.nsxh_mesh_vertices(h), (nv, self.dim), np.float64, copy=False)
        self.cells = _arr(L.nsxh_mesh_cells(h), (nc, self.dim + 1), np.int32, copy=False)
        self.bfaces = _arr(L.nsxh_mesh_bfaces(h), (nb, self.dim), np.int32)
        self.bface_ids = _arr(L.nsxh_mesh_bface_ids(h), (nb,), np.int32)
        self.bface_cells = _arr(L.nsxh_mesh_bface_cells(h), (nb,), np.int32)
        self.subdomain = _arr(L.nsxh_mesh_subdomain(h), (nc,), np.int32)

    @classmethod
    def cylinder(cls, dim, level=1, **kw):
        L = _lib()
        if kw:
            a = dict(m=4, nr=2, nxu=2, nxd=10, nyb=1, nyt=1, nz=4, grade_x=2.0, grade_r=2.0)
            a.update(kw)
            return cls(L.nsxh_mesh_cylinder(dim, a["m"], a["nr"], a["nxu"], a["nxd"], a["nyb"], a["nyt"], a["nz"],
                                            a["grade_x"], a["grade_r"]))
        return cls(L.nsxh_mesh_cylinder_level(dim, level))

    @classmethod
    def cube(cls, n):
        return cls(_lib().nsxh_mesh_cube(n))

    @classmethod
    def box(cls, dim, n, lo=None, hi=None):
        n = list(n) + [1] * (3 - len(n))
        lo = np.asarray(lo if lo is not None else [0.0] * dim, dtype=np.float64)
        hi = np.asarray(hi if hi is not None else [1.0] * dim, dtype=np.float64)
        return cls(_lib().nsxh_mesh_box(dim, n[0], n[1], n[2], lo.ctypes.data_as(_f64p), hi.ctypes.data_as(_f64p)))

    @classmethod
    def read_msh(cls, path):
        return cls(_lib().nsxh_mesh_read_msh(str(path).encode()))

    def partition(self, n_parts=1, n_sub=1, balance="cells"):
        fn = self._lib.nsxh_mesh_partition_owned if balance == "owned" else self._lib.nsxh_mesh_partition
        rc = fn(self._h, n_parts, n_sub)
        if rc != 0:
            raise ValueError("partition failed (rc=%d)" % rc)
        self.refresh()
        return self

    def __del__(self):
        try:
            self._lib.nsxh_mesh_free(self._h)
        except Exception:
            pass


class DoFs:

# ... 63 lines not shown
                         "send_u_ptr", "send_u_nodes", "send_p_ptr", "send_p_nodes"):
                f = getattr(L, "nsxh_rank_view_" + name)
                f.restype, f.argtypes = _i32p, [vp]
            L.nsxh_rank_view_cell_coords.restype = _f64p
            L.nsxh_rank_view_cell_coords.argtypes = [vp]
            L._rv_ready = True
        v = L.nsxh_rank_view_create(self._h, rank, world)
        if not v:
            raise ValueError("rank view needs n_subdomains to be a multiple of world")
        nc, nn, ns = L.nsxh_rank_view_n_cells(v), L.nsxh_rank_view_n_neighbors(v), L.nsxh_rank_view_n_virtual_ranks(v)
        out = {
            "rank": rank, "world": world, "n_cells": nc, "n_cells_layer1": L.nsxh_rank_view_n_cells_layer1(v),
            "cell_ids": _arr(L.nsxh_rank_view_cell_ids(v), (nc,), np.int32),
            "cell_dofs": _arr(L.nsxh_rank_view_cell_dofs(v), (nc, self.dofs_per_cell), np.int32),
            "cell_coords": _arr(L.nsxh_rank_view_cell_coords(v), (nc, self.dim + 1, self.dim), np.float64),
            "gpu_u_ptr": _arr(L.nsxh_rank_view_gpu_u_ptr(v), (world + 1,), np.int32),
            "gpu_p_ptr": _arr(L.nsxh_rank_view_gpu_p_ptr(v), (world + 1,), np.int32),
            "rank_u_ptr": _arr(L.nsxh_rank_view_rank_u_ptr(v), (ns + 1,), np.int32),
            "rank_p_ptr": _arr(L.nsxh_rank_view_rank_p_ptr(v), (ns + 1,), np.int32),
            "neighbors": _arr(L.nsxh_rank_view_neighbors(v), (nn,), np.int32),
            "send_u_ptr": _arr(L.nsxh_rank_view_send_u_ptr(v), (nn + 1,), np.int32),
            "send_p_ptr": _arr(L.nsxh_rank_view_send_p_ptr(v), (nn + 1,), np.int32),
        }
        out["send_u_nodes"] = _arr(L.nsxh_rank_view_send_u_nodes(v), (int(out["send_u_ptr"][-1]),), np.int32)
        out["send_p_nodes"] = _arr(L.nsxh_rank_view_send_p_nodes(v), (int(out["send_p_ptr"][-1]),), np.int32)
        L.nsxh_rank_view_free(v)
        return out

    def __del__(self):
        try:
            self._lib.nsxh_dofs_free(self._h)
        except Exception:
            pass


class Tables:

    CELL, FACE, HIGH = 0, 1, 2

    def __init__(self, dim, rule=0, order=0):
        L = _lib()
        h = L.nsxh_tables_create(dim, rule, order)
        if not h:
            raise ValueError("bad table request")
        self.dim = dim
        nq, n2, n1 = L.nsxh_tables_n_q(h), L.nsxh_tables_n_p2(h), L.nsxh_tables_n_p1(h)
        self.n_q, self.n_p2, self.n_p1, self.n_qf = nq, n2, n1, L.nsxh_tables_n_qf(h)
        self.points = _arr(L.nsxh_tables_points(h), (nq, dim), np.float64)
        self.weights = _arr(L.nsxh_tables_weights(h), (nq,), np.float64)
        self.N2 = _arr(L.nsxh_tables_N2(h), (nq, n2), np.float64)
        self.dN2 = _arr(L.nsxh_tables_dN2(h), (nq, n2, dim), np.float64)
        self.N1 = _arr(L.nsxh_tables_N1(h), (nq, n1), np.float64)
        self.dN1 = _arr(L.nsxh_tables_dN1(h), (nq, n1, dim), np.float64)
        L.nsxh_tables_free(h)


def ilu_stream_stats(rowptr, colind, block_ptr, blocks_per_wave=8, ncomp=3, gap=2, entries_per_tick=1):
    rp, ci, bp = (np.ascontiguousarray(a, dtype=np.int32) for a in (rowptr, colind, block_ptr))
    out = (C.c_int64 * 6)()
    rc = _lib().nsxh_ilu_stream_stats(len(rp) - 1, rp.ctypes.data_as(_i32p), ci.ctypes.data_as(_i32p), len(bp) - 1, bp.ctypes.data_as(_i32p),
                                      int(blocks_per_wave), int(ncomp), int(gap), int(entries_per_tick), out)
    if rc:
        raise ValueError("nsxh_ilu_stream_stats failed (%d)" % rc)
    keys = ("slabs", "max_wave_slabs", "in_block_nnz", "max_wave_rows", "waves", "used_slots")
    d = dict(zip(keys, (int(v) for v in out)))
    d["fill"] = d["used_slots"] / max(1, 64 * d["slabs"] * int(entries_per_tick))
    d["stream_bytes"] = d["slabs"] * 64 * (8 * int(entries_per_tick) + 4 * ((int(entries_per_tick) + 2) // 2))
    return d


def ilu_stream_apply(rowptr, colind, block_ptr, lu, b, ncomp=1, blocks_per_wave=8, gap=2, entries_per_tick=1, f32=False):
    rp, ci, bp = (np.ascontiguousarray(a, dtype=np.int32) for a in (rowptr, colind, block_ptr))
    lu, b = np.ascontiguousarray(lu, dtype=np.float64), np.ascontiguousarray(b, dtype=np.float64)
    x = np.empty_like(b)
    fn = _lib().nsxh_ilu_stream_apply_f32 if f32 else _lib().nsxh_ilu_stream_apply
    rc = fn(len(rp) - 1, rp.ctypes.data_as(_i32p), ci.ctypes.data_as(_i32p), len(bp) - 1, bp.ctypes.data_as(_i32p),
            int(blocks_per_wave), int(ncomp), int(gap), int(entries_per_tick), lu.ctypes.data_as(_f64p), b.ctypes.data_as(_f64p),
            x.ctypes.data_as(_f64p))
    if rc:
        raise ValueError("nsxh_ilu_stream_apply%s failed (%d)" % ("_f32" if f32 else "", rc))
    return x


def merge_ranks(ptr, max_rows):
    ptr = np.asarray(ptr)
    out = [int(ptr[0])]
    for k in range(1, len(ptr)):
        if ptr[k] - out[-1] > max_rows and ptr[k - 1] > out[-1]:
            out.append(int(ptr[k - 1]))
    if out[-1] != ptr[-1]:
        out.append(int(ptr[-1]))
    return np.array(out, dtype=np.int32)


def internal_layout(dofs, n_virtual, order="colour", schur_max_rows=0):
    L = _lib()
    cd = np.ascontiguousarray(dofs.cell_dofs, dtype=np.int32)
    cc = np.ascontiguousarray(dofs.cell_coords, dtype=np.float64)
    iu, ip = (np.ascontiguousarray(a, dtype=np.int32) for a in (dofs.owned_u_ptr, dofs.owned_p_ptr))
    cap = int(n_virtual) + len(iu) + 1
    perm2, perm1 = np.empty(dofs.n_nodes_p2, np.int32), np.empty(dofs.n_nodes_p1, np.int32)
    u_ptr, p_ptr, s_ptr = (np.empty(cap, np.int32) for _ in range(3))
    nr, ns, col = C.c_int32(), C.c_int32(), (C.c_int32 * 2)()
    rc = L.nsxh_internal_layout(dofs.dim, dofs.n_cells, dofs.dofs_per_cell, cd.ctypes.data_as(_i32p), cc.ctypes.data_as(_f64p), dofs.n_u, dofs.n_p,
                                len(iu) - 1, iu.ctypes.data_as(_i32p), ip.ctypes.data_as(_i32p), int(n_virtual), DoFs.ORDERINGS[order], int(schur_max_rows),
                                perm2.ctypes.data_as(_i32p), perm1.ctypes.data_as(_i32p), C.byref(nr), u_ptr.ctypes.data_as(_i32p),
                                p_ptr.ctypes.data_as(_i32p), C.byref(ns), s_ptr.ctypes.data_as(_i32p), col)
    if rc:
        raise ValueError("nsxh_internal_layout failed (%d)" % rc)
    return {"node_perm": perm2, "pnode_perm": perm1, "u_ptr": u_ptr[:nr.value + 1].copy(), "p_ptr": p_ptr[:nr.value + 1].copy(),
            "schur_ptr": s_ptr[:ns.value + 1].copy(), "colours": (int(col[0]), int(col[1]))}


class PermutedDoFs:

    def __init__(self, dofs, node_perm, pnode_perm, u_ptr, p_ptr):
        self.base, self.mesh = dofs, dofs.mesh
        self.dim, self.n_cells, self.dofs_per_cell = dofs.dim, dofs.n_cells, dofs.dofs_per_cell
        self.n_nodes_p2, self.n_nodes_p1, self.n_u, self.n_p, self.n_dofs = dofs.n_nodes_p2, dofs.n_nodes_p1, dofs.n_u, dofs.n_p, dofs.n_dofs
        self.node_perm, self.pnode_perm = np.asarray(node_perm, dtype=np.int64), np.asarray(pnode_perm, dtype=np.int64)
        dim = self.dim
        dmap = np.empty(self.n_dofs, dtype=np.int64)
        for c in range(dim):
            dmap[c:self.n_u:dim] = dim * self.node_perm + c
        dmap[self.n_u:] = self.n_u + self.pnode_perm
        self.dof_map = dmap
        self.cell_dofs = dmap[np.asarray(dofs.cell_dofs)].astype(np.int32)
        self.cell_coords = dofs.cell_coords
        sp = np.empty_like(np.asarray(dofs.support_points))
        sp[dmap] = dofs.support_points
        self.support_points = sp
        self.owned_u_ptr, self.owned_p_ptr = np.asarray(u_ptr, dtype=np.int32), np.asarray(p_ptr, dtype=np.int32)
        self.n_subdomains = len(self.owned_u_ptr) - 1
        self._ref = {}

    def to_new(self, x):
        out = np.empty_like(np.asarray(x, dtype=np.float64))
        out[self.dof_map] = x
        return out

    def to_old(self, y):
        return np.asarray(y)[self.dof_map]

    def boundary_dofs(self, boundary_id):
        return np.sort(self.dof_map[self.base.boundary_dofs(boundary_id)]).astype(np.int32)

    def reference_sparsity(self, block):
        if block not in self._ref:
            rp, ci = self.base.reference_sparsity(block)
            nu = self.n_u
            rmap = self.dof_map[:nu] if block in (0, 1) else self.dof_map[nu:] - nu
            cmap = self.dof_map[:nu] if block in (0, 2) else self.dof_map[nu:] - nu
            n = len(rp) - 1
            rows = np.repeat(np.arange(n), np.diff(rp))
            nr, ncol = rmap[rows], cmap[ci]
            order = np.lexsort((ncol, nr))
            cnt = np.bincount(nr, minlength=n)
            self._ref[block] = (np.concatenate(([0], np.cumsum(cnt))).astype(np.int32), ncol[order].astype(np.int32))
        return self._ref[block]
```

navierstokes_project_nm4pde_amd/host/frontend.cpp:

```cpp
#include "../../include/nsx_host.h"

#include <algorithm>
#include <array>
#include <cmath>
#include <cstdio>
#include <cstring>
#include <fstream>
#include <iomanip>
#include <map>
#include <numeric>
#include <sstream>
#include <string>
#include <unordered_map>
#include <vector>

#include <sys/stat.h>

#include "graph.hpp"
#include "ilu_stream.hpp"
#include "layout.hpp"

namespace {

const int TRI_LINES[3][2] = {{0, 1}, {1, 2}, {2, 0}};
const int TET_LINES[6][2] = {{0, 1}, {1, 2}, {2, 0}, {0, 3}, {1, 3}, {2, 3}};
const int TRI_FACES[3][2] = {{0, 1}, {1, 2}, {2, 0}};
const int TET_FACES[4][3] = {{0, 1, 2}, {1, 0, 3}, {0, 2, 3}, {2, 1, 3}};

inline uint64_t edge_key(int a, int b) {
  if (a > b) std::swap(a, b);
  return ((uint64_t)(uint32_t)a << 32) | (uint32_t)b;
}

}

struct nsxh_mesh {
  int dim = 0;
  std::vector<double> vertices;
  std::vector<int32_t> cells;
  std::vector<int32_t> bfaces, bface_ids, bface_cells;
  std::vector<int32_t> subdomain;
  int n_subdomains = 1;
  int n_vertices() const { return (int)(vertices.size() / dim); }
  int n_cells() const { return (int)(cells.size() / (dim + 1)); }
  int n_bfaces() const { return (int)bface_ids.size(); }
};

namespace {

double simplex_measure_signed(const nsxh_mesh &m, const int32_t *c) {
  const double *v = m.vertices.data();
  if (m.dim == 2) {
    const double *p0 = v + 2 * c[0], *p1 = v + 2 * c[1], *p2 = v + 2 * c[2];
    return 0.5 * ((p1[0] - p0[0]) * (p2[1] - p0[1]) - (p2[0] - p0[0]) * (p1[1] - p0[1]));
  }
  const double *p0 = v + 3 * c[0], *p1 = v + 3 * c[1], *p2 = v + 3 * c[2], *p3 = v + 3 * c[3];
  double a[3] = {p1[0] - p0[0], p1[1] - p0[1], p1[2] - p0[2]};
  double b[3] = {p2[0] - p0[0], p2[1] - p0[1], p2[2] - p0[2]};
  double d[3] = {p3[0] - p0[0], p3[1] - p0[1], p3[2] - p0[2]};
  return (a[0] * (b[1] * d[2] - b[2] * d[1]) - a[1] * (b[0] * d[2] - b[2] * d[0]) + a[2] * (b[0] * d[1] - b[1] * d[0])) / 6.0;
}

void orient_cells(nsxh_mesh &m) {
  const int nv = m.dim + 1;
  for (int c = 0; c < m.n_cells(); ++c) {
    int32_t *cc = m.cells.data() + (size_t)c * nv;
    if (simplex_measure_signed(m, cc) < 0) std::swap(cc[nv - 2], cc[nv - 1]);
  }
}

template <class F>
void extract_boundary(nsxh_mesh &m, F classify) {
  const int dim = m.dim, nv = dim + 1, nf = dim + 1;
  struct FaceRec {
    std::array<int32_t, 3> key;
    int32_t cell, lf;
  };
  std::vector<FaceRec> recs;
  recs.reserve((size_t)m.n_cells() * nf);
  for (int c = 0; c < m.n_cells(); ++c) {
    const int32_t *cc = m.cells.data() + (size_t)c * nv;
    for (int f = 0; f < nf; ++f) {
      FaceRec r;
      r.key = {-1, -1, -1};
      for (int k = 0; k < dim; ++k) r.key[k] = cc[dim == 2 ? TRI_FACES[f][k] : TET_FACES[f][k]];
      std::sort(r.key.begin(), r.key.begin() + dim);
      r.cell = c;
      r.lf = f;
      recs.push_back(r);
    }
  }
  std::sort(recs.begin(), recs.end(), [](const FaceRec &a, const FaceRec &b) {
    if (a.key != b.key) return a.key < b.key;
    return a.cell < b.cell;
  });
  struct BF {
    int32_t cell, lf;
  };
  std::vector<BF> bf;
  for (size_t i = 0; i < recs.size();) {
    size_t j = i + 1;
    while (j < recs.size() && recs[j].key == recs[i].key) ++j;
    if (j - i == 1) bf.push_back({recs[i].cell, recs[i].lf});
// ... 1145 lines not shown
        for (int a = 0; a < 3; ++a)
          for (int b = 0; b < 3; ++b) M[a][b] = b == j ? r[a] : J[a][b];
        lam[j] = (M[0][0] * (M[1][1] * M[2][2] - M[1][2] * M[2][1]) - M[0][1] * (M[1][0] * M[2][2] - M[1][2] * M[2][0]) +
                  M[0][2] * (M[1][0] * M[2][1] - M[1][1] * M[2][0])) / det;
      }
      double l0 = 1.0;
      bool inside = true;
      for (int j = 0; j < dim; ++j) {
        l0 -= lam[j];
        inside = inside && lam[j] >= -1e-12;
      }
      if (!inside || l0 < -1e-12) continue;
      const int32_t *cd = d->cell_dofs.data() + (size_t)c * d->dpc;
      double p = l0 * solution[cd[dim]];
      for (int j = 0; j < dim; ++j) p += lam[j] * solution[cd[(size_t)(dim + 1) * (j + 1) + dim]];
      val[k] = p;
      found[k] = true;
    }
  }
  *diff = val[0] - val[1];
  return (int)found[0] + (int)found[1];
}

}

namespace {
nsx::Csr csr_of(int n_rows, const int32_t *rowptr, const int32_t *colind) {
  nsx::Csr g;
  g.n_rows = g.n_cols = n_rows;
  g.rowptr.assign(rowptr, rowptr + n_rows + 1);
  g.colind.assign(colind, colind + rowptr[n_rows]);
  return g;
}
}

extern "C" int nsxh_ilu_stream_stats(int n_rows, const int32_t *rowptr, const int32_t *colind, int n_blocks, const int32_t *block_ptr,
                                     int blocks_per_wave, int ncomp, int gap, int entries_per_tick, int64_t out[6]) {
  if (!rowptr || !colind || !block_ptr || !out || n_rows < 0 || n_blocks < 1 || ncomp < 1 || gap < 1 || entries_per_tick < 1 || entries_per_tick > 4) return -1;
  try {
    nsx::IluStream s;
    nsx::build_ilu_stream(csr_of(n_rows, rowptr, colind), std::vector<int32_t>(block_ptr, block_ptr + n_blocks + 1), blocks_per_wave, ncomp, gap, s, entries_per_tick);
    out[0] = s.n_slabs, out[1] = s.max_wave_slabs, out[2] = s.in_block_nnz, out[3] = s.max_wave_rows, out[4] = s.n_waves, out[5] = s.used_slots;
    return s.ok ? 0 : -3;
  } catch (const std::exception &) {
    return -1;
  }
}

extern "C" int nsxh_ilu_stream_apply(int n_rows, const int32_t *rowptr, const int32_t *colind, int n_blocks, const int32_t *block_ptr,
                                     int blocks_per_wave, int ncomp, int gap, int entries_per_tick, const double *lu, const double *b, double *x) {
  if (!rowptr || !colind || !block_ptr || !lu || !b || !x || ncomp < 1 || gap < 1 || entries_per_tick < 1 || entries_per_tick > 4) return -1;
  try {
    const nsx::Csr g = csr_of(n_rows, rowptr, colind);
    const std::vector<int32_t> bptr(block_ptr, block_ptr + n_blocks + 1);
    nsx::IluStream s;
    nsx::build_ilu_stream(g, bptr, blocks_per_wave, ncomp, gap, s, entries_per_tick);
    if (!s.ok) return -3;
    nsx::replay_ilu_stream(g, bptr, s, lu, b, x);
    return 0;
  } catch (const std::exception &) {
    return -1;
  }
}

extern "C" int nsxh_ilu_stream_apply_f32(int n_rows, const int32_t *rowptr, const int32_t *colind, int n_blocks, const int32_t *block_ptr,
                                         int blocks_per_wave, int ncomp, int gap, int entries_per_tick, const double *lu, const double *b, double *x) {
  if (!rowptr || !colind || !block_ptr || !lu || !b || !x || ncomp < 1 || gap < 1 || entries_per_tick < 1 || entries_per_tick > 4) return -1;
  try {
    const nsx::Csr g = csr_of(n_rows, rowptr, colind);
    const std::vector<int32_t> bptr(block_ptr, block_ptr + n_blocks + 1);
    nsx::IluStream s;
    nsx::build_ilu_stream(g, bptr, blocks_per_wave, ncomp, gap, s, entries_per_tick);
    if (!s.ok) return -3;
    std::vector<double> lu32(lu, lu + g.nnz());
    for (int64_t q = 0; q < g.nnz(); ++q)
      if (s.slot_of[q] >= 0) lu32[q] = (double)(float)lu[q];
    nsx::replay_ilu_stream(g, bptr, s, lu32.data(), b, x);
    return 0;
  } catch (const std::exception &) {
    return -1;
  }
}

extern "C" int nsxh_internal_layout(int dim, int n_cells, int dofs_per_cell, const int32_t *cell_dofs, const double *cell_coords, int n_u, int n_p,
                                    int n_in_ranks, const int32_t *in_u_ptr, const int32_t *in_p_ptr, int n_virtual, int order, int schur_max_rows,
                                    int32_t *node_perm, int32_t *pnode_perm, int32_t *n_ranks, int32_t *u_ptr, int32_t *p_ptr, int32_t *n_schur,
                                    int32_t *schur_ptr, int32_t *colours) {
  if ((dim != 2 && dim != 3) || n_cells < 1 || !cell_dofs || !cell_coords || n_in_ranks < 1 || !in_u_ptr || !in_p_ptr || n_virtual < 1 || n_u % dim) return -1;
  const int nv = dim + 1, nl = dim == 2 ? 3 : 6, np2 = nv + nl;
  if (dofs_per_cell != nv * (dim + 1) + nl * dim) return -1;
  std::vector<int32_t> c2((size_t)n_cells * np2), c1((size_t)n_cells * nv);
  std::vector<double> cen((size_t)n_cells * dim, 0.0);
  for (int c = 0; c < n_cells; ++c) {
    const int32_t *cd = cell_dofs + (size_t)c * dofs_per_cell;
    for (int a = 0; a < np2; ++a) c2[(size_t)c * np2 + a] = cd[a < nv ? (dim + 1) * a : nv * (dim + 1) + dim * (a - nv)] / dim;
    for (int v = 0; v < nv; ++v) c1[(size_t)c * nv + v] = cd[(dim + 1) * v + dim] - n_u;
    for (int k = 0; k < nv; ++k)
      for (int d = 0; d < dim; ++d) cen[(size_t)c * dim + d] += cell_coords[((size_t)c * nv + k) * dim + d] / nv;
  }
  nsx::LayoutIn in;
  in.dim = dim;
  in.n_cells = n_cells;
  in.np2 = np2;
  in.np1 = nv;
  in.c2 = c2.data();
  in.c1 = c1.data();
  in.cen = cen.data();
  in.N2 = in.N2_all = n_u / dim;
  in.NP = n_p;
  in.in_u_ptr.assign(in_u_ptr, in_u_ptr + n_in_ranks + 1);
  in.in_p_ptr.assign(in_p_ptr, in_p_ptr + n_in_ranks + 1);
  nsx::LayoutOut out;
  nsx::build_layout(in, n_virtual, order, schur_max_rows, out);
  std::copy(out.perm2.begin(), out.perm2.end(), node_perm);
  std::copy(out.perm1.begin(), out.perm1.end(), pnode_perm);
  *n_ranks = (int32_t)out.u_ptr.size() - 1;
  std::copy(out.u_ptr.begin(), out.u_ptr.end(), u_ptr);
  std::copy(out.p_ptr.begin(), out.p_ptr.end(), p_ptr);
  const std::vector<int32_t> &sb = out.schur_ptr.empty() ? out.p_ptr : out.schur_ptr;
  *n_schur = (int32_t)sb.size() - 1;
  std::copy(sb.begin(), sb.end(), schur_ptr);
  if (colours) {
    colours[0] = out.n_colours;
    colours[1] = out.n_colours_p;
  }
  return 0;
}
```

navierstokes_project_nm4pde_amd/nsx.py:

```python
import ctypes as C

import numpy as np

from ._lib import DEV_SO, load

_i32p = C.POINTER(C.c_int32)
_f64p = C.POINTER(C.c_double)

TEMAM, DOUBLE_CONVECTION = 1, 2
YOSIDA, SIMPLE, AYOSIDA, ASIMPLE = 0, 1, 2, 3

API = [
    "nsx_create", "nsx_destroy", "nsx_last_error", "nsx_version", "nsx_set_tables", "nsx_set_mesh", "nsx_set_ranks",
    "nsx_set_schur_blocks", "nsx_set_solution", "nsx_get_solution", "nsx_get_solution_ghosted", "nsx_get_rhs",
    "nsx_set_rhs", "nsx_assemble", "nsx_assemble_time_step", "nsx_add_rhs", "nsx_apply_boundary_values",
    "nsx_solve_time_step", "nsx_prec_initialize", "nsx_prec_vmult", "nsx_system_vmult", "nsx_ilu_apply",
    "nsx_export_block", "nsx_schur_nnz", "nsx_schur_get", "nsx_scalar_graph_nnz", "nsx_scalar_graph", "nsx_ilu_get",
    "nsx_profile_enable", "nsx_profile_reset", "nsx_profile_count", "nsx_profile_get", "nsx_persistent_state", "nsx_path_info", "nsx_comm_self_halo_test", "nsx_comm_unique_id",
    "nsx_comm_init", "nsx_comm_init_callbacks", "nsx_comm_counters", "nsx_set_mesh_distributed", "nsx_set_force_faces", "nsx_compute_forces",
    "nsx_set_internal_layout", "nsx_layout_info", "nsx_layout_get", "nsx_gram_schmidt_cycle", "nsx_set_inner_precision",
    "nsx_gram_schmidt_sweeps", "nsx_compute_diagnostics", "nsx_get_cell_diagnostic", "nsx_schur_cg",
]
API_EXTRA = ["nsx_inner_F_vmult"]
FIRST_TOUCH, COLOUR, COLOUR_ALL = 0, 1, 2
# ... 113 lines not shown
    import torch.distributed as dist

    def allreduce(ctx, buf, count):
        t = torch.from_numpy(np.ctypeslib.as_array(buf, shape=(count,)))
        dist.all_reduce(t)
        return 0

    def exchange(ctx, n, ranks, send, scount, recv, rcount):
        reqs, keep = [], []
        for k in range(n):
            if rcount[k]:
                t = torch.from_numpy(np.ctypeslib.as_array(recv[k], shape=(rcount[k],)))
                keep.append(t)
                reqs.append(dist.irecv(t, src=int(ranks[k])))
            if scount[k]:
                t = torch.from_numpy(np.ctypeslib.as_array(send[k], shape=(scount[k],)).copy())
                keep.append(t)
                reqs.append(dist.isend(t, dst=int(ranks[k])))
        for q in reqs:
            q.wait()
        return 0

    return ALLREDUCE_FN(allreduce), EXCHANGE_FN(exchange)


class Nsx:

    def __init__(self, dofs, tables, nu, deltat, device=0, rank=0, world=1, comm="rccl", layout=None, inner_precision=None):
        L = lib()
        self.L = L
        self._h = C.c_void_p()
        prm = Params(dofs.dim, device, float(nu), float(deltat))
        rc = L.nsx_create(C.byref(prm), C.byref(self._h))
        if rc:
            raise NsxError(rc, (L.nsx_last_error(None) or b"").decode())
        self.dim, self.n_u, self.n_p = dofs.dim, dofs.n_u, dofs.n_p
        self.n = self.n_u + self.n_p
        self.dofs = dofs
        self.rank, self.world = rank, world
        N2, dN2, N1, w = _cd(tables.N2), _cd(tables.dN2), _cd(tables.N1), _cd(tables.weights)
        self._ck(L.nsx_set_tables(self._h, tables.n_q, tables.n_p2, tables.n_p1, _d(N2), _d(dN2), _d(N1), _d(w)))
        if inner_precision is not None:
            self.set_inner_precision(inner_precision)
        if layout:
            self.set_internal_layout(*layout)
        if world == 1:
            cd, cc = _ci(dofs.cell_dofs), _cd(dofs.cell_coords)
            self._ck(L.nsx_set_mesh(self._h, dofs.n_cells, dofs.dofs_per_cell, _i(cd), _d(cc), dofs.n_u, dofs.n_p))
            if dofs.n_subdomains > 1:
                self.set_ranks(dofs.owned_u_ptr, dofs.owned_p_ptr)
            return
        v = dofs.rank_view(rank, world)
        self.view = v
        cd, cc = _ci(v["cell_dofs"]), _cd(v["cell_coords"])
        arrs = [_ci(v[k]) for k in ("gpu_u_ptr", "gpu_p_ptr", "neighbors", "send_u_ptr", "send_u_nodes", "send_p_ptr", "send_p_nodes")]
        self._ck(L.nsx_set_mesh_distributed(self._h, v["n_cells"], v["n_cells_layer1"], dofs.dofs_per_cell, _i(cd), _d(cc),
                                            dofs.n_u, dofs.n_p, world, rank, _i(arrs[0]), _i(arrs[1]), len(arrs[2]), _i(arrs[2]),
                                            _i(arrs[3]), _i(arrs[4]), _i(arrs[5]), _i(arrs[6])))
        if len(v["rank_u_ptr"]) > 2:
            self.set_ranks(v["rank_u_ptr"], v["rank_p_ptr"])
        if comm == "callbacks":
            self._cb = gloo_callbacks()
            self._ck(L.nsx_comm_init_callbacks(self._h, rank, world, self._cb[0], self._cb[1], None))
        else:
            import torch.distributed as dist
            ident = (C.c_uint8 * 128)()
            if rank == 0:
                self._ck(L.nsx_comm_unique_id(ident))
            box = [bytes(ident)]
            dist.broadcast_object_list(box, src=0)
            ident = (C.c_uint8 * 128).from_buffer_copy(box[0])
            self._ck(L.nsx_comm_init(self._h, rank, world, ident))

    def persistent_state(self):
        st = (C.c_int * 4)()
        self._ck(self.L.nsx_persistent_state(self._h, st))
        return {"sweep_persistent": bool(st[0]), "cg_persistent": bool(st[1]), "fallbacks": int(st[2]), "dirty_mailbox_words": int(st[3])}

    PATH_KEYS = ("spmv_lds_staged", "spmv_chunks", "spmv_chunks_behind_halo", "sweep_entries_per_thread", "sweep_grid", "sweep_collective_inside",
                 "sweep_entries_per_thread_max", "cus_reserved", "schur_cg_path", "schur_blocks", "neighbours", "nodes_sent_per_exchange", "ghost_nodes",
                 "schur_dense_inverses", "sweep_off", "fallbacks", "rccl_sweep_velocity_plain", "rccl_sweep_velocity_masked", "rccl_sweep_block_plain",
                 "rccl_sweep_block_masked", "schur_blocks_per_partial", "sweep_velocity_one_gpu", "owned_p2_nodes", "owned_p1_nodes", "sweep_with_ilu_inside", "fused_launches",
                 "inner_F_fp32", "ilu_F_fp32", "schur_cg_rows_per_lane_group", "schur_cg_operator_in_lds")

    def path_info(self):
        v = (C.c_int * 32)()
        self._ck(self.L.nsx_path_info(self._h, v))
        return {k: int(v[i]) for i, k in enumerate(self.PATH_KEYS)}

    def comm_counters(self):
        c = (C.c_longlong * 2)()
        self._ck(self.L.nsx_comm_counters(self._h, c))
        return int(c[0]), int(c[1])

    def comm_self_halo_test(self, n_own, n_ghost, ncomp):
        e = C.c_double(0.0)
        self._ck(self.L.nsx_comm_self_halo_test(self._h, int(n_own), int(n_ghost), int(ncomp), C.byref(e)))
        return float(e.value)

    def comm_init_single(self):
        ident = (C.c_uint8 * 128)()
        self._ck(self.L.nsx_comm_unique_id(ident))
        self._ck(self.L.nsx_comm_init(self._h, 0, 1, ident))

    def gather_solution(self):
        x = np.zeros(self.n)
        self._ck(self.L.nsx_get_solution(self._h, _d(x)))
        if self.world > 1:
            import torch
            import torch.distributed as dist
            t = torch.from_numpy(x)
            if dist.get_backend() == "nccl":
                t = t.cuda()
            dist.all_reduce(t)
            x = t.cpu().numpy()
        return x

    def _ck(self, rc):
        if rc:
            raise NsxError(rc, (self.L.nsx_last_error(self._h) or b"").decode())

    def close(self):
        if self._h:
            self.L.nsx_destroy(self._h)
            self._h = None

    def __del__(self):
        try:
            self.close()
        except Exception:
            pass

    def set_ranks(self, u_ptr, p_ptr):
        u_ptr, p_ptr = _ci(u_ptr), _ci(p_ptr)
        self._ck(self.L.nsx_set_ranks(self._h, len(u_ptr) - 1, _i(u_ptr), _i(p_ptr)))

    def set_internal_layout(self, n_virtual_ranks, order=COLOUR, schur_max_rows=0):
        self._ck(self.L.nsx_set_internal_layout(self._h, int(n_virtual_ranks), int(order), int(schur_max_rows)))

    def set_inner_precision(self, precision):
        self._ck(self.L.nsx_set_inner_precision(self._h, int(precision)))

    def layout_info(self):
        info = (C.c_int * 5)()
        self._ck(self.L.nsx_layout_info(self._h, info))
        return {"on": bool(info[0]), "ranks": int(info[1]), "schur_blocks": int(info[2]), "colours": int(info[3]), "colours_p": int(info[4])}

    def layout(self):
        info = self.layout_info()
        if self.world == 1:
            n2, n1 = self.n_u // self.dim, self.n_p
        else:
            n2 = int(self.view["gpu_u_ptr"][self.rank + 1] - self.view["gpu_u_ptr"][self.rank])
            n1 = int(self.view["gpu_p_ptr"][self.rank + 1] - self.view["gpu_p_ptr"][self.rank])
        out = {"node_perm": np.empty(n2, np.int32), "pnode_perm": np.empty(n1, np.int32), "u_ptr": np.empty(info["ranks"] + 1, np.int32),
               "p_ptr": np.empty(info["ranks"] + 1, np.int32), "schur_ptr": np.empty(info["schur_blocks"] + 1, np.int32)}
        self._ck(self.L.nsx_layout_get(self._h, *[_i(out[k]) for k in ("node_perm", "pnode_perm", "u_ptr", "p_ptr", "schur_ptr")]))
        out.update(info)
        return out

    def set_schur_blocks(self, p_ptr):
        p_ptr = _ci(p_ptr)
        self._ck(self.L.nsx_set_schur_blocks(self._h, len(p_ptr) - 1, _i(p_ptr)))

    def set_solution(self, v):
        v = _cd(v)
        assert v.shape == (self.n,)
        self._ck(self.L.nsx_set_solution(self._h, _d(v)))

    def _get(self, fn):
        v = np.zeros(self.n)
# ... 174 lines not shown
```

Baseline: 14.46.

## Precompute a load-balanced Schur product plan and fuse preconditioner diagonal kernels

Adds a host-built plan for the Schur complement numeric product B D^-1 B^T. The plan precomputes the matching column pairs per entry, packs them into 16-bit items and balances them across 64 lanes per group of 8 rows, so the per-step merge walk is replaced by a software-pipelined gather kernel that uses LDS. It also fuses diagonal extraction, the reciprocals and the schur_w scaling into one kernel, skips the host sync when the Schur-input cache cannot be kept, and adds an LDS-based ILU block-inversion kernel. The cost is extra plan memory and setup time, and the plan is only used when rows fit its size limits.

```diff
diff --git a/include/nsx_host.h b/include/nsx_host.h
--- a/include/nsx_host.h
+++ b/include/nsx_host.h
@@ -108,6 +108,12 @@
 int nsxh_ilu_stream_apply_f32(int n_rows, const int32_t *rowptr, const int32_t *colind, int n_blocks, const int32_t *block_ptr,
                               int blocks_per_wave, int ncomp, int gap, int entries_per_tick, const double *lu, const double *b, double *x);
 
+void *nsxh_schur_plan_build(int n_rows_S, const int32_t *rowptr_S, const int32_t *colind_S, int n_rows_B, const int32_t *rowptr_B,
+                            const int32_t *colind_B, int rows_per_group, int max_row_len);
+int nsxh_schur_plan_info(const void *plan, int64_t out[10]);
+int nsxh_schur_plan_get(const void *plan, int32_t *grp, uint16_t *items, uint32_t *hdr, int32_t *lane_hdr, int32_t *lane_load);
+void nsxh_schur_plan_free(void *plan);
+
 int nsxh_internal_layout(int dim, int n_cells, int dofs_per_cell, const int32_t *cell_dofs, const double *cell_coords, int n_u, int n_p,
                          int n_in_ranks, const int32_t *in_u_ptr, const int32_t *in_p_ptr, int n_virtual, int order, int schur_max_rows,
                          int32_t *node_perm, int32_t *pnode_perm, int32_t *n_ranks, int32_t *u_ptr, int32_t *p_ptr, int32_t *n_schur,
diff --git a/navierstokes_project_nm4pde_amd/csrc/nsx_blas.hip b/navierstokes_project_nm4pde_amd/csrc/nsx_blas.hip
--- a/navierstokes_project_nm4pde_amd/csrc/nsx_blas.hip
+++ b/navierstokes_project_nm4pde_amd/csrc/nsx_blas.hip
@@ -421,6 +421,8 @@
     info[27] = h->ilu_F_fp32_used;
     info[28] = h->cg_last_rpg;
     info[29] = h->cg_last_lres;
+    info[30] = h->schur_last_path;
+    info[31] = h->ilu_invert_path;
   } catch (const nsx::Error &e) {
     h->err = e.msg;
     return e.code;
diff --git a/navierstokes_project_nm4pde_amd/csrc/nsx_internal.hpp b/navierstokes_project_nm4pde_amd/csrc/nsx_internal.hpp
--- a/navierstokes_project_nm4pde_amd/csrc/nsx_internal.hpp
+++ b/navierstokes_project_nm4pde_amd/csrc/nsx_internal.hpp
@@ -263,6 +263,15 @@
   nsx::DevBuf<double> schur_w_prev;
   bool schur_valid = false, schur_pending = false;
   int schur_type = -1;
+  struct {
+    bool ok = false, stale = true;
+    int n_groups = 0, max_lds_rows = 0;
+    nsx::DevBuf<int32_t> grp, lane_hdr;
+    nsx::DevBuf<uint16_t> items;
+    nsx::DevBuf<uint32_t> hdr;
+  } splan;
+  int schur_last_path = 0;
+  int ilu_invert_path = 0;
   std::vector<nsx::DevBuf<double> *> pool;
   nsx::DevBuf<double> red_partial;
   nsx::DevBuf<double> scal;
@@ -372,7 +381,6 @@
 void ilu_check(nsx_handle *h);
 bool ilu_solve(nsx_handle *h, const DevCsr &g, const IluSchedule &s, const double *lu, const double *b, double *x, int ncomp,
                const char *name, int dot_slot = -1, bool f32 = false, int *used_f32 = nullptr);
-void extract_diag(nsx_handle *h, const DevCsr &g, const double *vals, double *d);
 void abs_rowsum(nsx_handle *h, const DevCsr &g, const double *vals, double *d);
 
 struct Span {
diff --git a/navierstokes_project_nm4pde_amd/csrc/nsx_setup.hip b/navierstokes_project_nm4pde_amd/csrc/nsx_setup.hip
--- a/navierstokes_project_nm4pde_amd/csrc/nsx_setup.hip
+++ b/navierstokes_project_nm4pde_amd/csrc/nsx_setup.hip
@@ -5,6 +5,7 @@
 #include "nsx_internal.hpp"
 #include "../host/ilu_stream.hpp"
 #include "../host/layout.hpp"
+#include "../host/schur_plan.hpp"
 
 using namespace nsx;
 
@@ -385,6 +386,7 @@
     S.rowptr[i + 1] = (int32_t)S.colind.size();
   }
   h->gS.host = std::move(S);
+  h->splan.stale = true;
   upload_csr(h, h->gS, true);
   h->vSchur.alloc(h->gS.nnz());
   h->luS.alloc(h->gS.nnz());
@@ -403,6 +405,33 @@
   h->prec_ready = false;
   h->schur_valid = false;
   h->mgs.dist_fit.clear();
+}
+
+static void build_schur_plan_dev(nsx_handle *h) {
+  if (!h->splan.stale) return;
+  h->splan.stale = false;
+  h->splan.ok = false;
+  SchurPlan pl;
+  const int max_row = getenv("NSX_SCHUR_PLAN_MAXROW") ? atoi(getenv("NSX_SCHUR_PLAN_MAXROW")) : SCHUR_PLAN_MAX_ROW;
+  build_schur_plan(h->gS.host, h->gB.host, pl, SCHUR_PLAN_ROWS, max_row);
+  if (getenv("NSX_DEBUG")) {
+    if (pl.ok)
+      fprintf(stderr, "[nsx] schur plan: %d groups of %d rows, %lld entries, %lld matches in %lld trips of %d items (fill %.3f, longest lane %lld items), "
+                      "%.1f MB (items %.1f, headers %.1f), LDS rows <= %d\n",
+              pl.n_groups, SCHUR_PLAN_ROWS, (long long)pl.n_entries, (long long)pl.n_matches, (long long)pl.n_trips, SCHUR_PLAN_STEP,
+              (double)pl.n_matches / std::max<double>(1.0, (double)pl.n_trips * SCHUR_PLAN_LANES * SCHUR_PLAN_STEP), (long long)pl.max_lane_items,
+              1e-6 * pl.bytes(), 2e-6 * pl.items.size(), 4e-6 * pl.hdr.size(), pl.max_lds_rows);
+    else
+      fprintf(stderr, "[nsx] schur plan: not usable (%d), the merge walk stays\n", pl.why);
+  }
+  if (!pl.ok) return;
+  h->splan.n_groups = pl.n_groups;
+  h->splan.max_lds_rows = pl.max_lds_rows;
+  h->splan.grp.upload(pl.grp, h->stream);
+  h->splan.lane_hdr.upload(pl.lane_hdr, h->stream);
+  h->splan.items.upload(pl.items, h->stream);
+  h->splan.hdr.upload(pl.hdr, h->stream);
+  h->splan.ok = true;
 }
 
 void ensure_schedules(nsx_handle *h) {
@@ -416,6 +445,7 @@
   const bool denseS = !(getenv("NSX_DENSE_S") && atoi(getenv("NSX_DENSE_S")) == 0);
   setup_ilu_schedule(h, h->gS.host, sb, h->schedS, bpwS, denseS, 1);
   build_cg_plan(h);
+  build_schur_plan_dev(h);
   h->cgd_agreed = -1;
   h->sched_dirty = false;
 }
diff --git a/navierstokes_project_nm4pde_amd/csrc/nsx_solve.hip b/navierstokes_project_nm4pde_amd/csrc/nsx_solve.hip
--- a/navierstokes_project_nm4pde_amd/csrc/nsx_solve.hip
+++ b/navierstokes_project_nm4pde_amd/csrc/nsx_solve.hip
@@ -327,7 +327,7 @@
   const unsigned long long a = (unsigned long long)__double_as_longlong(w[i]), b = (unsigned long long)__double_as_longlong(prev[i]);
   if (a != b) {
     prev[i] = w[i];
-    __hip_atomic_store(changed, 1, __ATOMIC_RELAXED, __HIP_MEMORY_SCOPE_SYSTEM);
+    if (changed) __hip_atomic_store(changed, 1, __ATOMIC_RELAXED, __HIP_MEMORY_SCOPE_SYSTEM);
   }
 }
 static bool schur_inputs_unchanged(nsx_handle *h, int type) {
@@ -342,10 +342,28 @@
     return false;
   }
   comm_halo_u(h, h->schur_w.p);
+  const bool may_keep = cache && !h->comm;
   *flag = 0;
-  hipLaunchKernelGGL(k_same_and_keep, dim3(cdiv(n, 256)), dim3(256), 0, h->stream, n, h->schur_w.p, h->schur_w_prev.p, (int *)(h->pub_dev + N_SLOTS + 4));
+  hipLaunchKernelGGL(k_same_and_keep, dim3(cdiv(n, 256)), dim3(256), 0, h->stream, n, h->schur_w.p, h->schur_w_prev.p,
+                     may_keep ? (int *)(h->pub_dev + N_SLOTS + 4) : nullptr);
+  if (!may_keep) return false;
   HIP_CHECK(hipStreamSynchronize(h->stream));
-  return cache && !h->comm && *flag == 0;
+  return *flag == 0;
+}
+
+__global__ void k_prec_diagonals(int n, int dim, const int32_t *__restrict__ diag, const double *__restrict__ v, const double *__restrict__ lump,
+                                 const double *__restrict__ mask, double *__restrict__ D, double *__restrict__ D_inv,
+                                 double *__restrict__ neg_D_inv, double *__restrict__ w) {
+  const int i = blockIdx.x * blockDim.x + threadIdx.x;
+  if (i >= n) return;
+  const double d = v[diag[i / dim]], one = 1.0, neg = -1.0;
+  D[i] = d;
+  D_inv[i] = one / d;
+  const double nd = neg / d;
+  neg_D_inv[i] = nd;
+  double x = lump ? lump[i] : nd;
+  x *= mask[i];
+  w[i] = neg * x;
 }
 
 void prec_initialize(nsx_handle *h, int type) {
@@ -354,27 +372,29 @@
   HIP_CHECK(hipSetDevice(h->prm.device));
   const int n_u = h->n_u;
   const double *V = nullptr;
+  const double *vals = nullptr;
   if (type == NSX_PREC_YOSIDA) {
-    extract_diag(h, h->gA, h->vMass.p, h->diag_D.p);
+    vals = h->vMass.p;
   } else if (type == NSX_PREC_SIMPLE || type == NSX_PREC_ASIMPLE || type == NSX_PREC_AYOSIDA) {
-    extract_diag(h, h->gA, h->vF.p, h->diag_D.p);
+    vals = h->vF.p;
   } else {
     NSX_THROW(NSX_ERR_ARG, "Invalid preconditioner type");
   }
-  v_reciprocal(h, n_u, h->diag_D_inv.p, h->diag_D.p, 1.0);
-  v_reciprocal(h, n_u, h->neg_diag_D_inv.p, h->diag_D.p, -1.0);
-  V = h->neg_diag_D_inv.p;
   if (type == NSX_PREC_AYOSIDA) {
     abs_rowsum(h, h->gA, h->vMass.p, h->lump_M.p);
     v_reciprocal(h, n_u, h->lump_M.p, h->lump_M.p, -1.0);
     V = h->lump_M.p;
   }
-  v_copy(h, n_u, h->schur_w.p, V);
-  v_scale_vec(h, n_u, h->schur_w.p, h->dirmask.p);
-  v_scale(h, n_u, h->schur_w.p, -1.0);
+  {
+    LaunchScope ls(h, "prec_diagonals", 48.0 * n_u);
+    if (n_u > 0)
+      hipLaunchKernelGGL(k_prec_diagonals, dim3(cdiv(n_u, 256)), dim3(256), 0, h->stream, n_u, h->dim, h->gA.diag.p, vals, V, h->dirmask.p, h->diag_D.p,
+                         h->diag_D_inv.p, h->neg_diag_D_inv.p, h->schur_w.p);
+  }
   const bool f32 = h->inner_precision == NSX_INNER_FP32;
   if (f32) convert_F_f32(h);
   ilu_factor(h, h->gA, h->schedF, h->vF.p, h->luF.p, "ilu_factor_F", f32);
+  h->schur_last_path = 0;
   if (!schur_inputs_unchanged(h, type)) {
     h->schur_valid = false;
     h->schur_pending = true;
diff --git a/navierstokes_project_nm4pde_amd/csrc/nsx_sparse.hip b/navierstokes_project_nm4pde_amd/csrc/nsx_sparse.hip
--- a/navierstokes_project_nm4pde_amd/csrc/nsx_sparse.hip
+++ b/navierstokes_project_nm4pde_amd/csrc/nsx_sparse.hip
@@ -2,6 +2,7 @@
 
 #include "nsx_internal.hpp"
 #include "nsx_ilu_lanes.hpp"
+#include "../host/schur_plan.hpp"
 
 namespace nsx {
 
@@ -557,21 +558,12 @@
   if (n > 0) hipLaunchKernelGGL(k_to_f32, dim3(cdiv(n, 256)), dim3(256), 0, h->stream, n, h->vF.p, h->vF32.p, (int *)(h->pub_dev + N_SLOTS + 3));
 }
 
-__global__ void k_extract_diag(int n_nodes, int dim, const int32_t *__restrict__ diag, const double *__restrict__ v, double *__restrict__ d) {
-  const int i = blockIdx.x * blockDim.x + threadIdx.x;
-  if (i >= n_nodes * dim) return;
-  d[i] = v[diag[i / dim]];
-}
 __global__ void k_abs_rowsum(int n_nodes, int dim, const int32_t *__restrict__ rp, const double *__restrict__ v, double *__restrict__ d) {
   const int i = blockIdx.x * blockDim.x + threadIdx.x;
   if (i >= n_nodes) return;
   double s = 0.0;
   for (int p = rp[i]; p < rp[i + 1]; ++p) s += fabs(v[p]);
   for (int c = 0; c < dim; ++c) d[(size_t)i * dim + c] = s;
-}
-void extract_diag(nsx_handle *h, const DevCsr &g, const double *vals, double *d) {
-  LaunchScope ls(h, "extract_diag", 0);
-  hipLaunchKernelGGL(k_extract_diag, dim3(cdiv(h->n_u, 256)), dim3(256), 0, h->stream, g.n_rows(), h->dim, g.diag.p, vals, d);
 }
 void abs_rowsum(nsx_handle *h, const DevCsr &g, const double *vals, double *d) {
   LaunchScope ls(h, "abs_rowsum", 0);
@@ -612,14 +604,110 @@
   }
 }
 
+template <int DIM>
+struct SchurTrip {
+  double g[SCHUR_PLAN_STEP][DIM], r[SCHUR_PLAN_STEP][DIM];
+  int e[SCHUR_PLAN_STEP];
+  uint2 raw;
+};
+template <int DIM>
+__global__ __launch_bounds__(SCHUR_PLAN_LANES) void k_schur_plan(const int32_t *__restrict__ grp, const int32_t *__restrict__ lane_hdr,
+                                                                 const uint2 *__restrict__ items, const uint2 *__restrict__ hdr,
+                                                                 const int32_t *__restrict__ srp, const int32_t *__restrict__ brp,
+                                                                 const int32_t *__restrict__ bci, const double *__restrict__ bv,
+                                                                 const double *__restrict__ w, double *__restrict__ sv) {
+  extern __shared__ double rv[];
+  constexpr int L = SCHUR_PLAN_LANES, ST = SCHUR_PLAN_STEP;
+  const int g = blockIdx.x, lane = threadIdx.x;
+  const int r0 = grp[4 * g], t0 = grp[4 * g + 1], nt = grp[4 * g + 2], r1 = grp[4 * g + 4];
+  const int b0 = brp[r0], nb = brp[r1] - b0, e0 = srp[r0];
+  for (int t = lane; t < nb; t += L) {
+    const int k = bci[b0 + t];
+#pragma unroll
+    for (int c = 0; c < DIM; ++c) rv[t * DIM + c] = bv[(size_t)(b0 + t) * DIM + c] * w[(size_t)k * DIM + c];
+  }
+  __syncthreads();
+  if (nt == 0) return;
+  const uint2 *it0 = items + (size_t)t0 * L + lane;
+  int hk = lane_hdr[g * L + lane];
+  uint2 hn = hdr[hk];
+  int cur_e = e0, cur_ib = 0, cur_bj = 0;
+  bool fresh = true;
+  double acc = 0.0;
+  auto item = [](const uint2 &raw, int m) -> uint32_t { return ((m < 2 ? raw.x : raw.y) >> (16 * (m & 1))) & 0xffffu; };
+  auto issue = [&](SchurTrip<DIM> &T, const uint2 raw) {
+    T.raw = raw;
+#pragma unroll
+    for (int m = 0; m < ST; ++m) {
+      const uint32_t it = item(raw, m);
+      if (fresh && it != SCHUR_PLAN_SKIP) {
+        cur_e = e0 + (int)(hn.x & 0xfffffu);
+        cur_ib = (int)(hn.x >> 20);
+        cur_bj = (int)hn.y;
+        hn = hdr[++hk];
+        fresh = false;
+      }
+      T.e[m] = cur_e;
+      const double *gp = bv + (size_t)(cur_bj + (int)((it >> 7) & 127u)) * DIM;
+      const double *rp = rv + (cur_ib + (int)(it & 127u)) * DIM;
+#pragma unroll
+      for (int c = 0; c < DIM; ++c) {
+        T.g[m][c] = gp[c];
+        T.r[m][c] = rp[c];
+      }
+      if (it & SCHUR_PLAN_LAST) fresh = true;
+    }
+  };
+  auto consume = [&](const SchurTrip<DIM> &T) {
+#pragma unroll
+    for (int m = 0; m < ST; ++m) {
+      const uint32_t it = item(T.raw, m);
+      if (!(it & SCHUR_PLAN_SKIP)) {
+#pragma unroll
+        for (int c = 0; c < DIM; ++c) acc += T.r[m][c] * T.g[m][c];
+      }
+      if (it & SCHUR_PLAN_LAST) {
+        sv[T.e[m]] = acc;
+        acc = 0.0;
+      }
+    }
+  };
+  SchurTrip<DIM> A, B;
+  uint2 rb = it0[(size_t)min(1, nt - 1) * L];
+  issue(A, it0[0]);
+  for (int s = 0; s < nt; s += 2) {
+    const uint2 ra2 = it0[(size_t)min(s + 2, nt - 1) * L], rb2 = it0[(size_t)min(s + 3, nt - 1) * L];
+    if (s + 1 < nt) issue(B, rb);
+    consume(A);
+    if (s + 2 < nt) issue(A, ra2);
+    if (s + 1 < nt) consume(B);
+    rb = rb2;
+  }
+}
+
 void schur_numeric(nsx_handle *h, const double *w) {
   comm_halo_u(h, w);
+  const bool want_plan = !(getenv("NSX_SCHUR_PLAN") && atoi(getenv("NSX_SCHUR_PLAN")) == 0);
+  const size_t shm_plan = (size_t)h->splan.max_lds_rows * h->dim * sizeof(double);
+  LaunchScope ls(h, "schur_numeric", 0);
+  if (want_plan && h->splan.ok && h->splan.n_groups > 0 && shm_plan <= 64 * 1024) {
+    h->schur_last_path = 2;
+    const int ng = h->splan.n_groups;
+    const uint2 *items = reinterpret_cast<const uint2 *>(h->splan.items.p), *hdr = reinterpret_cast<const uint2 *>(h->splan.hdr.p);
+    if (h->dim == 2)
+      hipLaunchKernelGGL((k_schur_plan<2>), dim3(ng), dim3(SCHUR_PLAN_LANES), shm_plan, h->stream, h->splan.grp.p, h->splan.lane_hdr.p, items, hdr,
+                         h->gS.rowptr.p, h->gB.rowptr.p, h->gB.colind.p, h->vB.p, w, h->vSchur.p);
+    else
+      hipLaunchKernelGGL((k_schur_plan<3>), dim3(ng), dim3(SCHUR_PLAN_LANES), shm_plan, h->stream, h->splan.grp.p, h->splan.lane_hdr.p, items, hdr,
+                         h->gS.rowptr.p, h->gB.rowptr.p, h->gB.colind.p, h->vB.p, w, h->vSchur.p);
+    return;
+  }
+  h->schur_last_path = 1;
   int max_row = 0;
   const Csr &B = h->gB.host;
   for (int i = 0; i < B.n_rows; ++i) max_row = std::max(max_row, B.rowptr[i + 1] - B.rowptr[i]);
   const size_t shm = (size_t)max_row * (h->dim * 8 + 4) + 8;
   if (shm > 160 * 1024) NSX_THROW(NSX_ERR_UNSUPPORTED, "row of block(1,0) too long for the Schur kernel (%d)", max_row);
-  LaunchScope ls(h, "schur_numeric", 0);
   if (h->dim == 2)
     hipLaunchKernelGGL((k_schur<2>), dim3(h->NP), dim3(64), shm, h->stream, h->NP, h->gS.rowptr.p, h->gS.colind.p, h->gB.rowptr.p,
                        h->gB.colind.p, h->vB.p, w, max_row, h->vSchur.p);
@@ -735,6 +823,85 @@
         if (k < n) acc -= lu[p] * Ps[k * n + j];
       }
       Ps[i * n + j] = acc;
+    }
+  }
+  __syncthreads();
+  double *Pb = P + off[blk];
+  for (int q = threadIdx.x; q < n * n; q += 128) Pb[q] = Ps[q];
+}
+
+__host__ __device__ inline size_t ilu_invert_lds_bytes(int max_rows, int max_nz) {
+  const size_t nz = ((size_t)max_nz + 3) & ~(size_t)3;
+  return (size_t)max_rows * max_rows * 8 + nz * 10 + (size_t)(max_rows + 4) * 2 * 2;
+}
+__device__ __forceinline__ double invert_row_chain(const double *lv, const uint16_t *lc, const double *Pj, int n, int e0, int e1, double acc) {
+  int e = __builtin_amdgcn_readfirstlane(e0);
+  const int pe = __builtin_amdgcn_readfirstlane(e1);
+  if (e >= pe) return acc;
+  int k[8];
+  double l[8];
+#pragma unroll
+  for (int t = 0; t < 8; ++t) {
+    const int q = min(e + t, pe - 1);
+    k[t] = lc[q];
+    l[t] = lv[q];
+  }
+  while (true) {
+    double y[8];
+#pragma unroll
+    for (int t = 0; t < 8; ++t) y[t] = Pj[k[t] * n];
+    const int en = e + 8;
+    int kn[8];
+    double ln[8];
+#pragma unroll
+    for (int t = 0; t < 8; ++t) {
+      const int q = min(en + t, pe - 1);
+      kn[t] = lc[q];
+      ln[t] = lv[q];
+    }
+#pragma unroll
+    for (int t = 0; t < 8; ++t)
+      if (e + t < pe) acc -= l[t] * y[t];
+    if (en >= pe) return acc;
+    e = en;
+#pragma unroll
+    for (int t = 0; t < 8; ++t) {
+      k[t] = kn[t];
+      l[t] = ln[t];
+    }
+  }
+}
+__global__ __launch_bounds__(128) void k_ilu_invert_lds_factor(const int32_t *__restrict__ bptr, const int64_t *__restrict__ off,
+                                                               const int32_t *__restrict__ diag, const int32_t *__restrict__ in_lo,
+                                                               const int32_t *__restrict__ cptr, const int32_t *__restrict__ cpos,
+                                                               const int32_t *__restrict__ ci, const double *__restrict__ lu,
+                                                               double *__restrict__ P, int max_rows, int max_nz) {
+  extern __shared__ double lds_i[];
+  const int nzp = (max_nz + 3) & ~3, mr = max_rows + 4;
+  double *Ps = lds_i;
+  double *lv = lds_i + (size_t)max_rows * max_rows;
+  uint16_t *lc = (uint16_t *)(lv + nzp);
+  uint16_t *lrp = lc + nzp;
+  uint16_t *ldg = lrp + mr;
+  const int blk = blockIdx.x, r0 = bptr[blk], n = bptr[blk + 1] - r0;
+  if (n == 0) return;
+  const int j = threadIdx.x, c0 = cptr[r0], nzb = cptr[r0 + n] - c0;
+  for (int q = threadIdx.x; q <= n; q += 128) lrp[q] = (uint16_t)(cptr[r0 + q] - c0);
+  for (int q = threadIdx.x; q < n; q += 128) ldg[q] = (uint16_t)(cptr[r0 + q] - c0 + diag[r0 + q] - in_lo[r0 + q]);
+#pragma unroll 4
+  for (int e = threadIdx.x; e < nzb; e += 128) {
+    const int p = cpos[c0 + e];
+    lv[e] = lu[p];
+    lc[e] = (uint16_t)(ci[p] - r0);
+  }
+  __syncthreads();
+  if (j < n) {
+    const double *Pj = Ps + j;
+    for (int i = 0; i < n; ++i)
+      Ps[i * n + j] = invert_row_chain(lv, lc, Pj, n, lrp[i], ldg[i], i == j ? 1.0 : 0.0);
+    for (int i = n - 1; i >= 0; --i) {
+      const int pd = ldg[i];
+      Ps[i * n + j] = invert_row_chain(lv, lc, Pj, n, pd + 1, lrp[i + 1], lv[pd] * Ps[i * n + j]);
     }
   }
   __syncthreads();
@@ -1145,18 +1312,32 @@
   }
   if (s.dense) {
     LaunchScope ls(h, "ilu_invert", 8.0 * (double)s.dn_entries + 12.0 * g.nnz());
-    const bool inv_lds = !(getenv("NSX_ILU_INVERT_LDS") && atoi(getenv("NSX_ILU_INVERT_LDS")) == 0);
+    const int want = getenv("NSX_ILU_INVERT_LDS") ? atoi(getenv("NSX_ILU_INVERT_LDS")) : 2;
     const size_t shm = (size_t)s.max_rows * s.max_rows * sizeof(double);
-    if (inv_lds && s.max_rows <= 112) {
-      static bool attr_set = false;
-      if (!attr_set && shm > 64 * 1024) {
-        HIP_CHECK(hipFuncSetAttribute((const void *)k_ilu_invert_lds, hipFuncAttributeMaxDynamicSharedMemorySize, 112 * 112 * (int)sizeof(double)));
-        attr_set = true;
-      }
+    const size_t shm2 = ilu_invert_lds_bytes(s.max_rows, s.max_block_nnz);
+    const size_t budget = getenv("NSX_ILU_INVERT_LDS_BYTES") ? std::min<size_t>(160 * 1024, (size_t)std::max(0, atoi(getenv("NSX_ILU_INVERT_LDS_BYTES")))) : 160 * 1024;
+    auto allow_lds = [&](const void *fn, std::atomic<unsigned long long> &done, int bytes) {
+      const int dev = h->prm.device;
+      const unsigned long long bit = dev >= 0 && dev < 64 ? 1ull << dev : 0ull;
+      if (bit && (done.load() & bit)) return;
+      HIP_CHECK(hipFuncSetAttribute(fn, hipFuncAttributeMaxDynamicSharedMemorySize, bytes));
+      done.fetch_or(bit);
+    };
+    if (want >= 2 && s.max_rows <= 112 && s.max_block_nnz < 65535 && shm2 <= budget) {
+      static std::atomic<unsigned long long> done{0};
+      if (shm2 > 64 * 1024) allow_lds((const void *)k_ilu_invert_lds_factor, done, 160 * 1024);
+      hipLaunchKernelGGL(k_ilu_invert_lds_factor, dim3(s.n_blocks), dim3(128), shm2, h->stream, s.block_ptr.p, s.dn_off.p, g.diag.p, s.in_lo.p, s.in_cptr.p,
+                         s.in_cpos.p, g.colind.p, lu, s.dn_P.p, s.max_rows, (int)s.max_block_nnz);
+      h->ilu_invert_path = 2;
+    } else if (want >= 1 && s.max_rows <= 112) {
+      static std::atomic<unsigned long long> done{0};
+      if (shm > 64 * 1024) allow_lds((const void *)k_ilu_invert_lds, done, 112 * 112 * (int)sizeof(double));
       hipLaunchKernelGGL(k_ilu_invert_lds, dim3(s.n_blocks), dim3(128), shm, h->stream, s.block_ptr.p, s.dn_off.p, g.rowptr.p, g.colind.p, g.diag.p, lu, s.dn_P.p);
+      h->ilu_invert_path = 1;
     } else {
       hipLaunchKernelGGL(k_ilu_invert, dim3(s.n_blocks), dim3(256), 0, h->stream, s.block_ptr.p, s.dn_off.p, g.rowptr.p, g.colind.p, g.diag.p, lu,
                          s.dn_P.p);
+      h->ilu_invert_path = 0;
     }
   }
 }
diff --git a/navierstokes_project_nm4pde_amd/frontend.py b/navierstokes_project_nm4pde_amd/frontend.py
--- a/navierstokes_project_nm4pde_amd/frontend.py
+++ b/navierstokes_project_nm4pde_amd/frontend.py
@@ -69,6 +69,10 @@
         "nsxh_ilu_stream_stats": (C.c_int, [C.c_int, _i32p, _i32p, C.c_int, _i32p, C.c_int, C.c_int, C.c_int, C.c_int, C.POINTER(C.c_int64)]),
         "nsxh_ilu_stream_apply": (C.c_int, [C.c_int, _i32p, _i32p, C.c_int, _i32p, C.c_int, C.c_int, C.c_int, C.c_int, _f64p, _f64p, _f64p]),
         "nsxh_ilu_stream_apply_f32": (C.c_int, [C.c_int, _i32p, _i32p, C.c_int, _i32p, C.c_int, C.c_int, C.c_int, C.c_int, _f64p, _f64p, _f64p]),
+        "nsxh_schur_plan_build": (vp, [C.c_int, _i32p, _i32p, C.c_int, _i32p, _i32p, C.c_int, C.c_int]),
+        "nsxh_schur_plan_info": (C.c_int, [vp, C.POINTER(C.c_int64)]),
+        "nsxh_schur_plan_get": (C.c_int, [vp, vp, vp, vp, vp, vp]),
+        "nsxh_schur_plan_free": (None, [vp]),
         "nsxh_internal_layout": (C.c_int, [C.c_int, C.c_int, C.c_int, _i32p, _f64p, C.c_int, C.c_int, C.c_int, _i32p, _i32p, C.c_int, C.c_int, C.c_int,
                                            _i32p, _i32p, _i32p, _i32p, _i32p, _i32p, _i32p, _i32p]),
     }
@@ -298,6 +302,31 @@
     return x
 
 
+def schur_plan(rowptr_S, colind_S, rowptr_B, colind_B, rows_per_group=8, max_row_len=128):
+    srp, sci, brp, bci = (np.ascontiguousarray(a, dtype=np.int32) for a in (rowptr_S, colind_S, rowptr_B, colind_B))
+    L = _lib()
+    h = L.nsxh_schur_plan_build(len(srp) - 1, srp.ctypes.data_as(_i32p), sci.ctypes.data_as(_i32p), len(brp) - 1, brp.ctypes.data_as(_i32p),
+                                bci.ctypes.data_as(_i32p), int(rows_per_group), int(max_row_len))
+    if not h:
+        raise ValueError("nsxh_schur_plan_build failed")
+    try:
+        out = (C.c_int64 * 10)()
+        L.nsxh_schur_plan_info(h, out)
+        keys = ("ok", "why", "groups", "max_lds_rows", "entries", "matches", "trips", "max_lane_items", "headers", "bytes")
+        d = dict(zip(keys, (int(v) for v in out)))
+        d["ok"] = bool(d["ok"])
+        if d["ok"]:
+            d["grp"] = np.empty((d["groups"] + 1, 4), np.int32)
+            d["items"] = np.empty((d["trips"], 64, 4), np.uint16)
+            d["hdr"] = np.empty((d["headers"], 2), np.uint32)
+            d["lane_hdr"] = np.empty((d["groups"], 64), np.int32)
+            d["lane_load"] = np.empty((d["groups"], 64), np.int32)
+            L.nsxh_schur_plan_get(h, *[d[k].ctypes.data_as(C.c_void_p) for k in ("grp", "items", "hdr", "lane_hdr", "lane_load")])
+        return d
+    finally:
+        L.nsxh_schur_plan_free(h)
+
+
 def merge_ranks(ptr, max_rows):
     ptr = np.asarray(ptr)
     out = [int(ptr[0])]
diff --git a/navierstokes_project_nm4pde_amd/host/frontend.cpp b/navierstokes_project_nm4pde_amd/host/frontend.cpp
--- a/navierstokes_project_nm4pde_amd/host/frontend.cpp
+++ b/navierstokes_project_nm4pde_amd/host/frontend.cpp
@@ -19,6 +19,7 @@
 #include "graph.hpp"
 #include "ilu_stream.hpp"
 #include "layout.hpp"
+#include "schur_plan.hpp"
 
 namespace {
 
@@ -1330,6 +1331,36 @@
   }
 }
 
+extern "C" void *nsxh_schur_plan_build(int n_rows_S, const int32_t *rowptr_S, const int32_t *colind_S, int n_rows_B, const int32_t *rowptr_B,
+                                       const int32_t *colind_B, int rows_per_group, int max_row_len) {
+  if (!rowptr_S || !colind_S || !rowptr_B || !colind_B || n_rows_S < 0 || n_rows_B < 0 || rows_per_group < 1) return nullptr;
+  try {
+    nsx::SchurPlan *pl = new nsx::SchurPlan();
+    nsx::build_schur_plan(csr_of(n_rows_S, rowptr_S, colind_S), csr_of(n_rows_B, rowptr_B, colind_B), *pl, rows_per_group, max_row_len);
+    return pl;
+  } catch (const std::exception &) {
+    return nullptr;
+  }
+}
+extern "C" int nsxh_schur_plan_info(const void *plan, int64_t out[10]) {
+  if (!plan || !out) return -1;
+  const nsx::SchurPlan &pl = *static_cast<const nsx::SchurPlan *>(plan);
+  out[0] = pl.ok, out[1] = pl.why, out[2] = pl.n_groups, out[3] = pl.max_lds_rows, out[4] = pl.n_entries, out[5] = pl.n_matches, out[6] = pl.n_trips;
+  out[7] = pl.max_lane_items, out[8] = (int64_t)pl.hdr.size() / 2, out[9] = (int64_t)pl.bytes();
+  return 0;
+}
+extern "C" int nsxh_schur_plan_get(const void *plan, int32_t *grp, uint16_t *items, uint32_t *hdr, int32_t *lane_hdr, int32_t *lane_load) {
+  if (!plan) return -1;
+  const nsx::SchurPlan &pl = *static_cast<const nsx::SchurPlan *>(plan);
+  if (grp) std::copy(pl.grp.begin(), pl.grp.end(), grp);
+  if (items) std::copy(pl.items.begin(), pl.items.end(), items);
+  if (hdr) std::copy(pl.hdr.begin(), pl.hdr.end(), hdr);
+  if (lane_hdr) std::copy(pl.lane_hdr.begin(), pl.lane_hdr.end(), lane_hdr);
+  if (lane_load) std::copy(pl.lane_load.begin(), pl.lane_load.end(), lane_load);
+  return 0;
+}
+extern "C" void nsxh_schur_plan_free(void *plan) { delete static_cast<nsx::SchurPlan *>(plan); }
+
 extern "C" int nsxh_internal_layout(int dim, int n_cells, int dofs_per_cell, const int32_t *cell_dofs, const double *cell_coords, int n_u, int n_p,
                                     int n_in_ranks, const int32_t *in_u_ptr, const int32_t *in_p_ptr, int n_virtual, int order, int schur_max_rows,
                                     int32_t *node_perm, int32_t *pnode_perm, int32_t *n_ranks, int32_t *u_ptr, int32_t *p_ptr, int32_t *n_schur,
diff --git a/navierstokes_project_nm4pde_amd/host/schur_plan.hpp b/navierstokes_project_nm4pde_amd/host/schur_plan.hpp
--- /dev/null
+++ b/navierstokes_project_nm4pde_amd/host/schur_plan.hpp
@@ -0,0 +1,199 @@
+#pragma once
+#include <algorithm>
+#include <cstdint>
+#include <queue>
+#include <utility>
+#include <vector>
+
+#include "graph.hpp"
+
+namespace nsx {
+
+constexpr int SCHUR_PLAN_LANES = 64;
+constexpr int SCHUR_PLAN_ROWS = 8;
+constexpr int SCHUR_PLAN_STEP = 4;
+constexpr int SCHUR_PLAN_MAX_ROW = 128;
+constexpr uint16_t SCHUR_PLAN_SKIP = 0x4000u, SCHUR_PLAN_LAST = 0x8000u;
+
+struct SchurPlan {
+  bool ok = false;
+  int why = 0;
+  int n_groups = 0;
+  int max_lds_rows = 0;
+  int64_t n_entries = 0;
+  int64_t n_matches = 0;
+  int64_t n_trips = 0;
+  int64_t max_lane_items = 0;
+  std::vector<int32_t> grp;
+  std::vector<uint16_t> items;
+  std::vector<uint32_t> hdr;
+  std::vector<int32_t> lane_hdr;
+  std::vector<int32_t> lane_load;
+  size_t bytes() const { return grp.size() * 4 + items.size() * 2 + hdr.size() * 4 + lane_hdr.size() * 4; }
+};
+
+inline void build_schur_plan(const Csr &S, const Csr &B, SchurPlan &pl, int rows_per_group = SCHUR_PLAN_ROWS, int max_row_len = SCHUR_PLAN_MAX_ROW) {
+  constexpr int L = SCHUR_PLAN_LANES, ST = SCHUR_PLAN_STEP;
+  pl = SchurPlan();
+  const int n = S.n_rows, G = std::max(1, rows_per_group);
+  max_row_len = std::max(0, std::min(max_row_len, SCHUR_PLAN_MAX_ROW));
+  if (n <= 0 || S.nnz() == 0 || B.nnz() == 0 || B.n_rows < n || (int)S.rowptr.size() != n + 1 || (int)B.rowptr.size() != B.n_rows + 1) {
+    pl.why = 3;
+    return;
+  }
+  for (int64_t e = 0; e < S.nnz(); ++e)
+    if (S.colind[e] < 0 || S.colind[e] >= B.n_rows) {
+      pl.why = 3;
+      return;
+    }
+  for (int i = 0; i < B.n_rows; ++i)
+    if (B.rowptr[i + 1] - B.rowptr[i] > max_row_len) {
+      pl.why = 1;
+      return;
+    }
+  const int ng = (n + G - 1) / G;
+  for (int g = 0; g < ng; ++g) {
+    const int r0 = g * G, r1 = std::min(n, r0 + G);
+    if (B.rowptr[r1] - B.rowptr[r0] > 4096 || S.rowptr[r1] - S.rowptr[r0] >= (1 << 20)) {
+      pl.why = 2;
+      return;
+    }
+  }
+  pl.n_groups = ng;
+  pl.n_entries = S.nnz();
+  pl.grp.assign((size_t)(ng + 1) * 4, 0);
+  pl.lane_load.assign((size_t)ng * L, 0);
+  pl.lane_hdr.assign((size_t)ng * L, 0);
+  pl.hdr.assign((size_t)(S.nnz() + 1) * 2, 0u);
+  int64_t n_hdr = 0;
+  struct Entry {
+    int32_t e, i, cnt, first;
+  };
+  std::vector<Entry> ent;
+  std::vector<uint16_t> match;
+  std::vector<std::vector<int32_t>> of_lane(L);
+  for (int g = 0; g < ng; ++g) {
+    const int r0 = g * G, r1 = std::min(n, r0 + G);
+    pl.max_lds_rows = std::max(pl.max_lds_rows, B.rowptr[r1] - B.rowptr[r0]);
+    ent.clear();
+    match.clear();
+    for (int i = r0; i < r1; ++i) {
+      const int32_t *ci = B.colind.data() + B.rowptr[i];
+      const int ni = B.rowptr[i + 1] - B.rowptr[i];
+      for (int e = S.rowptr[i]; e < S.rowptr[i + 1]; ++e) {
+        const int j = S.colind[e];
+        const int32_t *cj = B.colind.data() + B.rowptr[j];
+        const int nj = B.rowptr[j + 1] - B.rowptr[j];
+        Entry en{e, i, 0, (int32_t)match.size()};
+        for (int p = 0, q = 0; p < nj; ++p) {
+          while (q < ni && ci[q] < cj[p]) ++q;
+          if (q < ni && ci[q] == cj[p]) {
+            match.push_back((uint16_t)(q | (p << 7)));
+            ++en.cnt;
+          }
+        }
+        ent.push_back(en);
+      }
+    }
+    std::vector<int32_t> order(ent.size());
+    for (size_t k = 0; k < ent.size(); ++k) order[k] = (int32_t)k;
+    std::stable_sort(order.begin(), order.end(), [&](int32_t a, int32_t b) { return ent[a].cnt > ent[b].cnt; });
+    typedef std::pair<int64_t, int> Load;
+    std::priority_queue<Load, std::vector<Load>, std::greater<Load>> pq;
+    for (int l = 0; l < L; ++l) {
+      pq.push(Load(0, l));
+      of_lane[l].clear();
+    }
+    for (int32_t k : order) {
+      Load t = pq.top();
+      pq.pop();
+      of_lane[t.second].push_back(k);
+      t.first += std::max(1, ent[k].cnt);
+      pq.push(t);
+    }
+    int64_t longest = 0;
+    for (int l = 0; l < L; ++l) {
+      int64_t load = 0;
+      for (int32_t k : of_lane[l]) load += std::max(1, ent[k].cnt);
+      pl.lane_load[(size_t)g * L + l] = (int32_t)load;
+      longest = std::max(longest, load);
+    }
+    const int64_t trips = (longest + ST - 1) / ST, t0 = pl.n_trips;
+    pl.max_lane_items = std::max(pl.max_lane_items, longest);
+    pl.grp[(size_t)g * 4 + 0] = r0;
+    pl.grp[(size_t)g * 4 + 1] = (int32_t)t0;
+    pl.grp[(size_t)g * 4 + 2] = (int32_t)trips;
+    pl.grp[(size_t)g * 4 + 3] = (int32_t)n_hdr;
+    pl.items.resize((size_t)(t0 + trips) * L * ST, SCHUR_PLAN_SKIP);
+    for (int l = 0; l < L; ++l) {
+      int64_t at = 0;
+      pl.lane_hdr[(size_t)g * L + l] = (int32_t)n_hdr;
+      for (size_t k = 0; k < of_lane[l].size(); ++k) {
+        const Entry &en = ent[of_lane[l][k]];
+        uint32_t *hw = pl.hdr.data() + (size_t)(n_hdr++) * 2;
+        hw[0] = (uint32_t)(en.e - S.rowptr[r0]) | ((uint32_t)(en.cnt ? B.rowptr[en.i] - B.rowptr[r0] : 0) << 20);
+        hw[1] = (uint32_t)(en.cnt ? B.rowptr[S.colind[en.e]] : 0);
+        const int cnt = std::max(1, en.cnt);
+        for (int m = 0; m < cnt; ++m, ++at) {
+          uint16_t it = en.cnt ? match[en.first + m] : SCHUR_PLAN_SKIP;
+          if (m == cnt - 1) it |= SCHUR_PLAN_LAST;
+          pl.items[((size_t)(t0 + at / ST) * L + l) * ST + at % ST] = it;
+        }
+        pl.n_matches += en.cnt;
+      }
+    }
+    pl.n_trips += trips;
+  }
+  pl.grp[(size_t)ng * 4 + 0] = n;
+  pl.grp[(size_t)ng * 4 + 1] = (int32_t)pl.n_trips;
+  pl.grp[(size_t)ng * 4 + 3] = (int32_t)n_hdr;
+  pl.hdr[(size_t)n_hdr * 2 + 1] = (uint32_t)B.rowptr[0];
+  if (pl.n_trips * L >= (int64_t)1 << 31) {
+    pl = SchurPlan();
+    pl.why = 2;
+    return;
+  }
+  pl.ok = true;
+}
+
+template <class Visit>
+inline bool replay_schur_plan(const Csr &S, const Csr &B, const SchurPlan &pl, Visit visit) {
+  constexpr int L = SCHUR_PLAN_LANES, ST = SCHUR_PLAN_STEP;
+  if (!pl.ok) return false;
+  std::vector<int32_t> pi, pj;
+  for (int g = 0; g < pl.n_groups; ++g) {
+    const int32_t *gr = pl.grp.data() + (size_t)g * 4;
+    const int r0 = gr[0], t0 = gr[1], nt = gr[2];
+    for (int l = 0; l < L; ++l) {
+      int k = pl.lane_hdr[(size_t)g * L + l];
+      const int k1 = l + 1 < L ? pl.lane_hdr[(size_t)g * L + l + 1] : gr[7];
+      bool fresh = true;
+      uint32_t w0 = 0, w1 = 0;
+      pi.clear();
+      pj.clear();
+      for (int64_t at = 0; at < (int64_t)nt * ST; ++at) {
+        const uint16_t it = pl.items[((size_t)(t0 + at / ST) * L + l) * ST + at % ST];
+        if (fresh && it != SCHUR_PLAN_SKIP) {
+          if (k >= k1) return false;
+          w0 = pl.hdr[(size_t)k * 2], w1 = pl.hdr[(size_t)k * 2 + 1];
+          ++k;
+          fresh = false;
+        }
+        if (!(it & SCHUR_PLAN_SKIP)) {
+          pi.push_back(B.rowptr[r0] + (int32_t)(w0 >> 20) + (it & 127));
+          pj.push_back((int32_t)w1 + ((it >> 7) & 127));
+        }
+        if (it & SCHUR_PLAN_LAST) {
+          visit(S.rowptr[r0] + (int32_t)(w0 & 0xfffffu), pi.data(), pj.data(), (int)pi.size());
+          pi.clear();
+          pj.clear();
+          fresh = true;
+        }
+      }
+      if (!pi.empty() || !fresh || k != k1) return false;
+    }
+  }
+  return true;
+}
+
+}
diff --git a/navierstokes_project_nm4pde_amd/nsx.py b/navierstokes_project_nm4pde_amd/nsx.py
--- a/navierstokes_project_nm4pde_amd/nsx.py
+++ b/navierstokes_project_nm4pde_amd/nsx.py
@@ -219,11 +219,12 @@
                  "schur_dense_inverses", "sweep_off", "fallbacks", "rccl_sweep_velocity_plain", "rccl_sweep_velocity_masked", "rccl_sweep_block_plain",
                  "rccl_sweep_block_masked", "schur_blocks_per_partial", "sweep_velocity_one_gpu", "owned_p2_nodes", "owned_p1_nodes", "sweep_with_ilu_inside", "fused_launches",
                  "inner_F_fp32", "ilu_F_fp32", "schur_cg_rows_per_lane_group", "schur_cg_operator_in_lds")
+    PATH_KEYS_SETUP = ("schur_product_path", "ilu_invert_path")
 
     def path_info(self):
         v = (C.c_int * 32)()
         self._ck(self.L.nsx_path_info(self._h, v))
-        return {k: int(v[i]) for i, k in enumerate(self.PATH_KEYS)}
+        return {k: int(v[i]) for i, k in enumerate(self.PATH_KEYS + self.PATH_KEYS_SETUP)}
 
     def comm_counters(self):
         c = (C.c_longlong * 2)()
```

After: 14.63, median of 6. 1.01x the previous value.
